# TimZaman/dotaclient

Hardware: NVIDIA H100
Metric: optimizer_steps_per_sec (higher is better)
Workload: dtype f32

## Files before the change

dotaclient_b200/_lib.py:

```python
import ctypes
import os

_HERE = os.path.dirname(os.path.abspath(__file__))
LIB_PATH = os.path.join(_HERE, "libdotaclient_b200.so")

_c = ctypes
_vp, _i32, _i64, _f32, _f64, _sz = _c.c_void_p, _c.c_int, _c.c_int64, _c.c_float, _c.c_double, _c.c_size_t
_ptr5 = _c.c_void_p * 5


class GatherDesc(_c.Structure):
    _fields_ = [("src", _vp), ("dst", _vp), ("outer", _i64), ("src_cols", _i64), ("row_bytes", _i64)]

SIGNATURES = {
    "dc_version": (_i32, []),
    "dc_last_error": (_c.c_char_p, []),
    "dc_device_info": (_i32, [_c.POINTER(_i32)] * 3),
    "dc_gae_scan": (_i32, [_vp, _i32, _vp, _vp, _i32, _vp, _vp, _f64, _f64, _vp, _vp, _vp]),
    "dc_vtrace_scan": (_i32, [_vp, _i32, _vp, _vp, _vp, _vp, _i32, _vp, _vp, _f64, _f64, _f64, _f64, _vp, _vp, _vp, _vp]),
    "dc_gather_columns": (_i32, [_c.POINTER(GatherDesc), _i32, _vp, _i64, _vp]),
    "dc_rnn_workspace_bytes": (_sz, [_i32, _i32, _i32]),
    "dc_rnn_seq_fwd": (_i32, [_i32, _vp, _vp, _vp, _vp, _vp, _i32, _i32, _i32, _vp, _vp]),
    "dc_rnn_seq_bwd": (_i32, [_i32, _vp, _vp, _vp, _vp, _vp, _vp, _vp, _vp, _vp, _i32, _i32, _i32, _vp, _vp]),
    "dc_rnn_seq_fwd_reset": (_i32, [_i32, _vp, _vp, _vp, _vp, _vp, _vp, _vp, _vp, _i32, _i32, _i32, _i32, _vp, _vp]),
    "dc_rnn_seq_bwd_reset": (_i32, [_i32, _vp, _vp, _vp, _vp, _vp, _vp, _vp, _vp, _vp, _vp, _vp, _i32, _i32, _i32, _i32, _vp,
                                    _vp]),
    "dc_gemm_tf32x3_supported": (_i32, [_i64, _i32, _i32]),
    "dc_gemm_tf32x3": (_i32, [_vp, _i32, _vp, _i32, _vp, _vp, _i32, _i64, _i32, _i32, _i32, _vp]),
    "dc_gemm_wgrad_workspace_bytes": (_sz, [_i32, _i32]),
    "dc_gemm_wgrad_tf32x3": (_i32, [_vp, _i32, _vp, _i32, _i64, _i32, _i32, _vp, _i32, _vp, _i32, _vp, _vp]),
    "dc_unit_basic_bwd_workspace_bytes": (_sz, []),
    "dc_env_fwd": (_i32, [_vp, _vp, _vp, _vp, _i32, _i64, _vp]),
    "dc_env_bwd_workspace_bytes": (_sz, []),
    "dc_env_bwd": (_i32, [_vp, _vp, _i32, _vp, _vp, _vp, _i64, _vp, _vp]),
    "dc_unit_wgrad_routed": (_i32, [_vp, _vp, _i32, _vp, _vp, _i64, _i32, _vp, _vp, _vp, _vp]),
    "dc_unit_dgrad_fused": (_i32, [_vp, _vp, _i32, _vp, _vp, _i32, _vp, _vp, _vp, _vp, _vp, _i64, _i32, _vp, _vp, _i32, _vp, _vp]),
    "dc_gemm_unit_max": (_i32, [_vp, _vp, _vp, _vp, _vp, _i32, _vp, _i64, _i32, _vp]),
    "dc_unit_embed_fwd": (_i32, [_vp, _vp, _vp, _vp, _vp, _vp, _vp, _vp, _i32, _vp, _i64, _i32, _vp]),
    "dc_target_unit_q_fwd": (_i32, [_vp, _i32, _c.c_void_p * 6, _vp, _vp, _vp, _i64, _vp]),
    "dc_target_unit_q_bwd": (_i32, [_vp, _c.c_void_p * 6, _vp, _vp, _vp, _i32, _i64, _vp]),
    "dc_ppo_loss_fwd_bwd": (_i32, [_ptr5, _ptr5, _ptr5, _vp, _vp, _vp, _vp, _i64, _f32, _f32, _f32, _ptr5, _vp, _vp,
                                   _vp, _vp, _vp]),
    "dc_ppo_loss_fwd_bwd_strided": (_i32, [_ptr5, _c.c_int64 * 5, _ptr5, _ptr5, _vp, _vp, _vp, _vp, _i64, _i64, _f32, _f32, _f32,
                                           _ptr5, _c.c_int64 * 5, _vp, _i64, _vp, _vp, _vp, _vp]),
    "dc_ppo_loss_fwd_bwd_dev": (_i32, [_ptr5, _c.c_int64 * 5, _ptr5, _ptr5, _vp, _vp, _vp, _vp, _i64, _vp, _i64, _vp,
                                       _ptr5, _c.c_int64 * 5, _vp, _i64, _vp, _vp, _vp, _vp, _vp]),
    "dc_ppo_loss_fwd_bwd_masked": (_i32, [_ptr5, _c.c_int64 * 5, _ptr5, _ptr5, _vp, _vp, _vp, _vp, _i64, _vp, _vp, _i64,
                                          _vp, _ptr5, _c.c_int64 * 5, _vp, _i64, _vp, _vp, _vp, _vp, _vp]),
    "dc_ppo_loss_fwd_bwd_joint": (_i32, [_ptr5, _c.c_int64 * 5, _ptr5, _ptr5, _vp, _vp, _vp, _vp, _i64, _vp, _vp, _i64,
                                         _vp, _ptr5, _c.c_int64 * 5, _vp, _i64, _vp, _vp, _vp, _vp, _vp]),
    "dc_selected_logp": (_i32, [_ptr5, _ptr5, _ptr5, _i64, _vp, _vp]),
    "dc_select_actions": (_i32, [_ptr5, _c.c_int64 * 5, _ptr5, _vp, _i64, _vp, _vp, _vp]),
    "dc_grad_flags": (_i32, [_vp, _i64, _vp, _i32, _vp, _vp]),
    "dc_grad_finish": (_i32, [_vp, _vp, _vp, _vp, _vp, _vp, _vp, _vp, _i32, _i64, _f64, _f64, _f64, _f64, _f64, _vp, _vp,
                              _vp, _vp]),
    "dc_grad_finish_dev": (_i32, [_vp, _vp, _vp, _vp, _vp, _vp, _vp, _vp, _i32, _i64, _vp, _f64, _f64, _f64, _vp, _vp, _vp,
                                  _vp]),
}

PPO_WORKSPACE_BYTES = 512
FINISH_WORKSPACE_BYTES = 1024
LOSS_SLOTS = 16
HPARAM_SLOTS = 8
HP_LR, HP_E_CLIP, HP_ENTROPY_COEF, HP_VF_COEF, HP_MAX_GRAD_NORM, HP_VALUE_CLIP = range(6)
PPO_STATS_SLOTS = 16
STAT_APPROX_KL, STAT_CLIP_FRACTION, STAT_EXPLAINED_VAR = 0, 6, 12
STAT_JOINT_APPROX_KL, STAT_JOINT_CLIP_FRACTION = 13, 14
VTRACE_STATS_SLOTS = 8
GATHER_MAX_TENSORS = 32
MAX_PARAM_TENSORS = 96

_lib = None


class NativeLibraryError(RuntimeError):
    pass


def load():
    global _lib
    if _lib is not None:
        return _lib
    if not os.path.exists(LIB_PATH):
        raise NativeLibraryError(
            "%s not found: build it with `python -m dotaclient_b200.build` (needs nvcc, sm_90a). "
            "dotaclient_b200 has no CPU fallback." % LIB_PATH)
    lib = ctypes.CDLL(LIB_PATH)
    for name, (res, args) in SIGNATURES.items():
        try:
            fn = getattr(lib, name)
        except AttributeError:
            continue
        fn.restype = res
        fn.argtypes = args
    _lib = lib
    return lib


def exported(name):
    lib = load()
    return hasattr(lib, name)


def check(rc, what):
    if rc != 0:
        msg = load().dc_last_error()
        raise RuntimeError("%s failed (code %d): %s" % (what, rc, msg.decode() if msg else "?"))


def ptr(t):
    return None if t is None else t.data_ptr()


def ptr5(tensors):
    return _ptr5(*[t.data_ptr() if t is not None else None for t in tensors])


def stream_ptr():
    import torch
    return torch.cuda.current_stream().cuda_stream
```

dotaclient_b200/csrc/capi.cu:

```cuda
#include <cstdarg>
#include <cstdio>
#include "dc_common.cuh"

static thread_local char g_err[512] = "";

void dc_set_error(const char *fmt, ...) {
    va_list ap;
    va_start(ap, fmt);
    vsnprintf(g_err, sizeof(g_err), fmt, ap);
    va_end(ap);
}

int dc_sm_count() {
    static int cached[64] = {0};
    int dev = 0;
    if (cudaGetDevice(&dev) != cudaSuccess || dev < 0 || dev >= 64) return 132;
    if (cached[dev] == 0) {
        int n = 0;
        if (cudaDeviceGetAttribute(&n, cudaDevAttrMultiProcessorCount, dev) != cudaSuccess || n <= 0) n = 132;
        cached[dev] = n;
    }
    return cached[dev];
}

extern "C" {

int dc_version(void) { return 107; }

const char *dc_last_error(void) { return g_err; }

int dc_device_info(int *sm_count, int *cc_major, int *cc_minor) {
    int dev = 0;
    DC_CUDA(cudaGetDevice(&dev));
    int v = 0;
    if (sm_count) { DC_CUDA(cudaDeviceGetAttribute(&v, cudaDevAttrMultiProcessorCount, dev)); *sm_count = v; }
    if (cc_major) { DC_CUDA(cudaDeviceGetAttribute(&v, cudaDevAttrComputeCapabilityMajor, dev)); *cc_major = v; }
    if (cc_minor) { DC_CUDA(cudaDeviceGetAttribute(&v, cudaDevAttrComputeCapabilityMinor, dev)); *cc_minor = v; }
    return DC_OK;
}

}
```

dotaclient_b200/csrc/gemm_tf32x3.cu:

```cuda
#include "dc_common.cuh"
#include "unit_basic.cuh"

namespace {

constexpr int BM = 128, BN = 128, BK = 32;
constexpr int kStages = 2;
constexpr int kTileBytes = BM * BK * 4;
constexpr int kStageBytes = 4 * kTileBytes;
constexpr int kProducerThreads = 128;
constexpr int kProducerGroups = kStages;
constexpr int kConsumerWarp0 = 4 * kProducerGroups;
constexpr int kConsumerThreads = 256;
constexpr int kThreads = kConsumerWarp0 * 32 + kConsumerThreads;
constexpr int kLdS = BN + 8;
constexpr int kDIn = kUnitFeatures;
constexpr size_t kOffStaging = (size_t)kStages * kStageBytes;
constexpr size_t kOffUnits = kOffStaging + (size_t)BM * kLdS * 4;
constexpr size_t kOffBars = kOffUnits + (size_t)BM * kDIn * 4;
constexpr size_t kSmemBytes = kOffBars + 128 + 1024 ;

#define DC_ACC8(b) "+f"(d[b]), "+f"(d[b + 1]), "+f"(d[b + 2]), "+f"(d[b + 3]), "+f"(d[b + 4]), "+f"(d[b + 5]), "+f"(d[b + 6]), "+f"(d[b + 7])
__device__ __forceinline__ void wgmma_m64n128k8(float (&d)[64], uint64_t desc_a, uint64_t desc_b) {
    asm volatile(
        "{\n\t.reg .pred p;\n\tsetp.ne.b32 p, %66, 0;\n\t"
        "wgmma.mma_async.sync.aligned.m64n128k8.f32.tf32.tf32 "
        "{%0, %1, %2, %3, %4, %5, %6, %7, %8, %9, %10, %11, %12, %13, %14, %15, "
        "%16, %17, %18, %19, %20, %21, %22, %23, %24, %25, %26, %27, %28, %29, %30, %31, "
        "%32, %33, %34, %35, %36, %37, %38, %39, %40, %41, %42, %43, %44, %45, %46, %47, "
        "%48, %49, %50, %51, %52, %53, %54, %55, %56, %57, %58, %59, %60, %61, %62, %63}, "
        "%64, %65, p, 1, 1;\n\t}\n"
        : DC_ACC8(0), DC_ACC8(8), DC_ACC8(16), DC_ACC8(24), DC_ACC8(32), DC_ACC8(40), DC_ACC8(48), DC_ACC8(56)
        : "l"(desc_a), "l"(desc_b), "r"(1));
}
#undef DC_ACC8

__device__ __forceinline__ void mma_stage(float (&d)[64], uint32_t stage_base, int wg) {
    const uint64_t a_hi = dc_wgmma_desc(stage_base + wg * (64 * 128)), a_lo = dc_wgmma_desc(stage_base + kTileBytes + wg * (64 * 128));
    const uint64_t b_hi = dc_wgmma_desc(stage_base + 2 * kTileBytes), b_lo = dc_wgmma_desc(stage_base + 3 * kTileBytes);
#pragma unroll
    for (int i = 0; i < 64; ++i) dc_reg_fence(d[i]);
    dc_wgmma_fence();
#pragma unroll
    for (int ks = 0; ks < BK / 8; ++ks) {
        const uint64_t adv = (uint64_t)(ks * 2);
        wgmma_m64n128k8(d, a_lo + adv, b_hi + adv);
        wgmma_m64n128k8(d, a_hi + adv, b_lo + adv);
        wgmma_m64n128k8(d, a_hi + adv, b_hi + adv);
    }
    dc_wgmma_commit();
    dc_wgmma_wait0();
#pragma unroll
    for (int i = 0; i < 64; ++i) dc_reg_fence(d[i]);
}

__device__ __forceinline__ void consume(float (&d)[64], unsigned char *tiles, uint64_t *full, uint64_t *empty, uint32_t &c, int n,
                                       int wg, int lane) {
#pragma unroll
    for (int i = 0; i < 64; ++i) d[i] = 0.f;
    for (int kc = 0; kc < n; ++kc, ++c) {
        const int s = c % kStages;
        dc_mbar_wait(&full[s], (c / kStages) & 1);
        __syncwarp();
        mma_stage(d, dc_smem_u32(tiles + (size_t)s * kStageBytes), wg);
        __syncwarp();
        if (lane == 0) dc_mbar_arrive(&empty[s]);
    }
}

__device__ __forceinline__ void consumer_sync() { asm volatile("bar.sync 1, %0;" ::"n"(kConsumerThreads) : "memory"); }

__device__ __forceinline__ void stage_acc(const float (&d)[64], float *S, int ct) {
    const int wg = ct >> 7, w = (ct >> 5) & 3, lane = ct & 31;
    const int r0 = 64 * wg + 16 * w + (lane >> 2), c0 = 2 * (lane & 3);
#pragma unroll
    for (int i = 0; i < 64; i += 2) {
        const int row = r0 + 8 * ((i >> 1) & 1), col = 8 * (i >> 2) + c0;
        *reinterpret_cast<float2 *>(S + row * kLdS + col) = make_float2(d[i], d[i + 1]);
    }
}

__device__ __forceinline__ void init_ring(uint64_t *bars) {
    if (threadIdx.x == 0) {
        for (int s = 0; s < kStages; ++s) { dc_mbar_init(&bars[s], 4); dc_mbar_init(&bars[kStages + s], kConsumerThreads / 32); }
        asm volatile("fence.mbarrier_init.release.cluster;" ::: "memory");
    }
    __syncthreads();
}
__device__ __forceinline__ unsigned char *smem_base(unsigned char *raw) {
    return reinterpret_cast<unsigned char *>((reinterpret_cast<uintptr_t>(raw) + 1023) & ~(uintptr_t)1023);
}
template <typename F>
__device__ __forceinline__ void produce(uint64_t *full, uint64_t *empty, uint32_t c, int lane, F &&store) {
    const int s = c % kStages;
    dc_mbar_wait(&empty[s], ((c / kStages) & 1) ^ 1);
    store(s);
    asm volatile("fence.proxy.async.shared::cta;" ::: "memory");
    __syncwarp();
    if (lane == 0) dc_mbar_arrive(&full[s]);
}

__device__ __forceinline__ void tile_load_k(const float *__restrict__ src, int ld, int row0, int rows_total, int k0, int t,
                                            float4 (&v)[8]) {
    const int c = t & 7, r0 = t >> 3;
#pragma unroll
    for (int i = 0; i < 8; ++i) {
        const int r = r0 + 16 * i;
        v[i] = (row0 + r < rows_total) ? __ldg(reinterpret_cast<const float4 *>(src + (size_t)(row0 + r) * ld + k0) + c)
                                       : make_float4(0.f, 0.f, 0.f, 0.f);
    }
}
__device__ __forceinline__ void tile_store_k(const float4 (&v)[8], unsigned char *dst_hi, unsigned char *dst_lo, int t) {
    const int c = t & 7, r0 = t >> 3;
#pragma unroll
    for (int i = 0; i < 8; ++i) {
        const int r = r0 + 16 * i;
        const int off = r * 128 + ((c ^ (r & 7)) << 4);
        float4 hi, lo;
        hi.x = dc_tf32_rna(v[i].x); hi.y = dc_tf32_rna(v[i].y); hi.z = dc_tf32_rna(v[i].z); hi.w = dc_tf32_rna(v[i].w);
        lo.x = v[i].x - hi.x; lo.y = v[i].y - hi.y; lo.z = v[i].z - hi.z; lo.w = v[i].w - hi.w;
        *reinterpret_cast<float4 *>(dst_hi + off) = hi;
        *reinterpret_cast<float4 *>(dst_lo + off) = lo;
    }
}

template <int NU>
struct DembRaw {
    static constexpr int kP = NU == 16 ? 1 : 2;
    static constexpr int kU = NU == 16 ? 8 : NU;
    float4 d[kP], d2[kP], a[kP];
    uint32_t am[kP];
    float g[kP][kU];
    bool ok[kP];
};
template <>
struct DembRaw<1> {
    float4 v[8];
};

template <int NU>
__device__ __forceinline__ void demb_fetch(DembRaw<NU> &raw, const float *__restrict__ dx, const float *__restrict__ dx2, int ld_dx,
                                           const uint8_t *__restrict__ argmax, const float *__restrict__ dl, int ld_dl,
                                           const float *__restrict__ att, int tok0, int n_tok, int k0, int t) {
    const float4 zero4 = make_float4(0.f, 0.f, 0.f, 0.f);
    if constexpr (NU == 1) {
        const int c = t & 7, r0 = t >> 3;
#pragma unroll
        for (int i = 0; i < 8; ++i) {
            const int n = tok0 + r0 + 16 * i;
            const bool ok = n < n_tok;
            const size_t nn = (size_t)min(n, n_tok - 1);
            float4 d = dx != nullptr ? __ldg(reinterpret_cast<const float4 *>(dx + nn * ld_dx + k0) + c) : zero4;
            if (dx2 != nullptr) {
                const float4 d2 = __ldg(reinterpret_cast<const float4 *>(dx2 + nn * ld_dx + k0) + c);
                d.x += d2.x; d.y += d2.y; d.z += d2.z; d.w += d2.w;
            }
            const float4 a4 = dl != nullptr ? __ldg(reinterpret_cast<const float4 *>(att + nn * 128 + k0) + c) : zero4;
            const float gl = dl != nullptr ? __ldg(dl + nn * ld_dl) : 0.f;
            raw.v[i] = ok ? make_float4(fmaf(gl, a4.x, d.x), fmaf(gl, a4.y, d.y), fmaf(gl, a4.z, d.z), fmaf(gl, a4.w, d.w)) : zero4;
        }
    } else {
        constexpr int kTileToks = (BM - BM % NU) / NU;
#pragma unroll
        for (int k = 0; k < DembRaw<NU>::kP; ++k) {
            const int p = t + kProducerThreads * k;
            const int c = p & 7, tokl = NU == 16 ? p >> 4 : p >> 3;
            const int u0 = NU == 16 ? ((p >> 3) & 1) * 8 : 0;
            const bool active = tokl < kTileToks;
            const int n = tok0 + tokl;
            raw.ok[k] = active && n < n_tok;
            const size_t nn = (size_t)min(n, n_tok - 1);
            float4 d = (active && dx != nullptr) ? __ldg(reinterpret_cast<const float4 *>(dx + nn * ld_dx + k0) + c) : zero4;
            const float4 d2 = (active && dx2 != nullptr) ? __ldg(reinterpret_cast<const float4 *>(dx2 + nn * ld_dx + k0) + c) : zero4;
            if constexpr (NU == 16) {
                raw.d2[k] = d2;
            } else {
                d.x += d2.x; d.y += d2.y; d.z += d2.z; d.w += d2.w;
            }
            raw.d[k] = d;
            raw.am[k] = (active && dx != nullptr) ? __ldg(reinterpret_cast<const uint32_t *>(argmax + nn * 128 + k0) + c) : 0u;
            raw.a[k] = (active && dl != nullptr) ? __ldg(reinterpret_cast<const float4 *>(att + nn * 128 + k0) + c) : zero4;
#pragma unroll
            for (int j = 0; j < DembRaw<NU>::kU; ++j) raw.g[k][j] = (active && dl != nullptr) ? __ldg(dl + nn * ld_dl + u0 + j) : 0.f;
        }
    }
}

__device__ __forceinline__ void store_hi_lo(unsigned char *dst_hi, unsigned char *dst_lo, int off, float4 o) {
    float4 hi, lo;
    hi.x = dc_tf32_rna(o.x); hi.y = dc_tf32_rna(o.y); hi.z = dc_tf32_rna(o.z); hi.w = dc_tf32_rna(o.w);
    lo.x = o.x - hi.x; lo.y = o.y - hi.y; lo.z = o.z - hi.z; lo.w = o.w - hi.w;
    *reinterpret_cast<float4 *>(dst_hi + off) = hi;
    *reinterpret_cast<float4 *>(dst_lo + off) = lo;
}

template <int NU>
__device__ __forceinline__ void demb_store(const DembRaw<NU> &raw, unsigned char *dst_hi, unsigned char *dst_lo, int t) {
    if constexpr (NU == 1) {
        tile_store_k(raw.v, dst_hi, dst_lo, t);
    } else {
        constexpr int kTileRows = BM - BM % NU, kTileToks = kTileRows / NU;
        const float4 zero4 = make_float4(0.f, 0.f, 0.f, 0.f);
#pragma unroll
        for (int k = 0; k < DembRaw<NU>::kP; ++k) {
            const int p = t + kProducerThreads * k;
            const int c = p & 7, tokl = NU == 16 ? p >> 4 : p >> 3;
            const int u0 = NU == 16 ? ((p >> 3) & 1) * 8 : 0;
            if (tokl < kTileToks) {
                float4 d = raw.d[k];
                if constexpr (NU == 16) { d.x += raw.d2[k].x; d.y += raw.d2[k].y; d.z += raw.d2[k].z; d.w += raw.d2[k].w; }
                const float4 a = raw.a[k];
                const uint32_t am = raw.am[k];
#pragma unroll
                for (int j = 0; j < DembRaw<NU>::kU; ++j) {
                    const int u = u0 + j, r = tokl * NU + u;
                    const float gl = raw.g[k][j];
                    float4 o;
                    o.x = fmaf(gl, a.x, (int)(am & 0xffu) == u ? d.x : 0.f);
                    o.y = fmaf(gl, a.y, (int)((am >> 8) & 0xffu) == u ? d.y : 0.f);
                    o.z = fmaf(gl, a.z, (int)((am >> 16) & 0xffu) == u ? d.z : 0.f);
                    o.w = fmaf(gl, a.w, (int)(am >> 24) == u ? d.w : 0.f);
                    store_hi_lo(dst_hi, dst_lo, r * 128 + ((c ^ (r & 7)) << 4), raw.ok[k] ? o : zero4);
                }
            }
        }
        if constexpr (kTileRows < BM) {
            if (t < (BM - kTileRows) * 8) {
                const int r = kTileRows + (t >> 3), c = t & 7;
                store_hi_lo(dst_hi, dst_lo, r * 128 + ((c ^ (r & 7)) << 4), zero4);
            }
        }
    }
}

__device__ __forceinline__ void store_row_k(const float (&v)[32], unsigned char *dst_hi, unsigned char *dst_lo, int row) {
#pragma unroll
    for (int c = 0; c < 8; ++c) {
        const int off = row * 128 + ((c ^ (row & 7)) << 4);
        float4 hi, lo;
        hi.x = dc_tf32_rna(v[4 * c]); hi.y = dc_tf32_rna(v[4 * c + 1]); hi.z = dc_tf32_rna(v[4 * c + 2]); hi.w = dc_tf32_rna(v[4 * c + 3]);
        lo.x = v[4 * c] - hi.x; lo.y = v[4 * c + 1] - hi.y; lo.z = v[4 * c + 2] - hi.z; lo.w = v[4 * c + 3] - hi.w;
        *reinterpret_cast<float4 *>(dst_hi + off) = hi;
        *reinterpret_cast<float4 *>(dst_lo + off) = lo;
    }
}

__global__ void __launch_bounds__(kThreads, 1) gemm_tf32x3_kernel(const float *__restrict__ A, int lda,
                                                                  const float *__restrict__ B, int ldb,
                                                                  const float *__restrict__ bias, float *__restrict__ C,
                                                                  int ldc, int M, int N, int K, int relu, int ksplit,
                                                                  long long c_split_stride) {
    constexpr int kTileRows = BM;
    extern __shared__ unsigned char smem_raw[];
    unsigned char *tiles = smem_base(smem_raw);
    float *S = reinterpret_cast<float *>(tiles + kOffStaging);
    uint64_t *full = reinterpret_cast<uint64_t *>(tiles + kOffBars), *empty = full + kStages;

    const int warp = threadIdx.x >> 5, lane = threadIdx.x & 31;
    const int m_blocks = (M + kTileRows - 1) / kTileRows, n_blocks = (N + BN - 1) / BN, k_chunks = K / BK / ksplit;
    const int tiles_mn = m_blocks * n_blocks, tiles_total = tiles_mn * ksplit;
    init_ring(full);

    if (warp < kConsumerWarp0) {
        const int t = threadIdx.x & (kProducerThreads - 1), g = warp >> 2;
        uint32_t c = 0;
        for (int tile = blockIdx.x; tile < tiles_total; tile += gridDim.x) {
            const int tmn = tile % tiles_mn, kc0 = (tile / tiles_mn) * k_chunks;
            const int m0 = (tmn / n_blocks) * kTileRows, n0 = (tmn % n_blocks) * BN;
            for (int kc = 0; kc < k_chunks; ++kc, ++c) {
                if ((int)(c % kProducerGroups) != g) continue;
                float4 va[8], vb[8];
                tile_load_k(A, lda, m0, M, (kc0 + kc) * BK, t, va);
                tile_load_k(B, ldb, n0, N, (kc0 + kc) * BK, t, vb);
                produce(full, empty, c, lane, [&](int s) {
                    unsigned char *st = tiles + (size_t)s * kStageBytes;
                    tile_store_k(va, st, st + kTileBytes, t);
                    tile_store_k(vb, st + 2 * kTileBytes, st + 3 * kTileBytes, t);
                });
            }
        }
    } else {
        const int ct = threadIdx.x - kConsumerWarp0 * 32, wg = ct >> 7, cw = ct >> 5;
        float d[64];
        uint32_t c = 0;
        for (int tile = blockIdx.x; tile < tiles_total; tile += gridDim.x) {
            const int tmn = tile % tiles_mn, sp = tile / tiles_mn;
            const int m0 = (tmn / n_blocks) * kTileRows, n0 = (tmn % n_blocks) * BN;
            consume(d, tiles, full, empty, c, k_chunks, wg, lane);
            consumer_sync();
            stage_acc(d, S, ct);
            consumer_sync();
            const bool lane_in = n0 + 4 * lane < N;
            const bool has_bias = bias != nullptr && sp == 0 && lane_in;
            const float4 b4 = has_bias ? __ldg(reinterpret_cast<const float4 *>(bias + n0) + lane) : make_float4(0.f, 0.f, 0.f, 0.f);
            float *cbase = C + (size_t)sp * (size_t)c_split_stride + n0 + 4 * lane;
            for (int r = cw; lane_in && r < BM && m0 + r < M; r += kConsumerThreads / 32) {
                float4 v = *reinterpret_cast<const float4 *>(S + r * kLdS + 4 * lane);
                if (has_bias) { v.x += b4.x; v.y += b4.y; v.z += b4.z; v.w += b4.w; }
                if (relu) { v.x = fmaxf(v.x, 0.f); v.y = fmaxf(v.y, 0.f); v.z = fmaxf(v.z, 0.f); v.w = fmaxf(v.w, 0.f); }
                *reinterpret_cast<float4 *>(cbase + (size_t)(m0 + r) * ldc) = v;
            }
        }
    }
}

constexpr int kWsRows = 64;
constexpr int kWsStages = 8;
constexpr int kWsChunkBytes = kWsRows * BK * 4;
constexpr int kWsThreads = kConsumerThreads + 128;
constexpr int kWsLdS = 40;
constexpr size_t kWsOffRing = (size_t)4 * 2 * kTileBytes;
constexpr size_t kWsOffStaging = kWsOffRing + (size_t)kWsStages * kWsChunkBytes;
constexpr size_t kWsOffBars = kWsOffStaging + (size_t)(kConsumerThreads / 32) * 16 * kWsLdS * 4;
constexpr size_t kWsSmemBytes = kWsOffBars + 2 * kWsStages * 8 + 1024 ;
constexpr size_t kWsOffUnits = kWsOffBars + 2 * kWsStages * 8;
constexpr size_t kWsGenSmemBytes = kWsOffUnits + (size_t)4 * kWsRows * kDIn * 4 + 1024 ;
static_assert(kWsSmemBytes <= 227 * 1024 && kWsGenSmemBytes <= 227 * 1024, "weight-stationary GEMM exceeds the shared-memory opt-in");
static_assert(kWsOffUnits % 16 == 0, "unit rows are staged with 16-byte stores");

struct GenA {
    const float *units, *w_b, *b_b;
    float *basic_out;
};

__device__ __forceinline__ void cp_async16(uint32_t dst, const void *src, uint32_t src_bytes) {
    asm volatile("cp.async.cg.shared.global [%0], [%1], 16, %2;" ::"r"(dst), "l"(src), "r"(src_bytes) : "memory");
}
__device__ __forceinline__ void cp_async_arrive(uint64_t *bar) {
    asm volatile("cp.async.mbarrier.arrive.noinc.shared::cta.b64 [%0];" ::"r"(dc_smem_u32(bar)) : "memory");
}

#define DC_ACC8(b) "+f"(d[b]), "+f"(d[b + 1]), "+f"(d[b + 2]), "+f"(d[b + 3]), "+f"(d[b + 4]), "+f"(d[b + 5]), "+f"(d[b + 6]), "+f"(d[b + 7])
__device__ __forceinline__ void wgmma_m64n128k8_rs(float (&d)[64], uint32_t a0, uint32_t a1, uint32_t a2, uint32_t a3, uint64_t desc_b) {
    asm volatile(
        "{\n\t.reg .pred p;\n\tsetp.ne.b32 p, %69, 0;\n\t"
        "wgmma.mma_async.sync.aligned.m64n128k8.f32.tf32.tf32 "
        "{%0, %1, %2, %3, %4, %5, %6, %7, %8, %9, %10, %11, %12, %13, %14, %15, "
        "%16, %17, %18, %19, %20, %21, %22, %23, %24, %25, %26, %27, %28, %29, %30, %31, "
        "%32, %33, %34, %35, %36, %37, %38, %39, %40, %41, %42, %43, %44, %45, %46, %47, "
        "%48, %49, %50, %51, %52, %53, %54, %55, %56, %57, %58, %59, %60, %61, %62, %63}, "
        "{%64, %65, %66, %67}, %68, p, 1, 1;\n\t}\n"
        : DC_ACC8(0), DC_ACC8(8), DC_ACC8(16), DC_ACC8(24), DC_ACC8(32), DC_ACC8(40), DC_ACC8(48), DC_ACC8(56)
        : "r"(a0), "r"(a1), "r"(a2), "r"(a3), "l"(desc_b), "r"(1));
}
#undef DC_ACC8

__device__ __forceinline__ void ws_fetch(float (&v)[16], const float *chunk, int rlo, int rhi, bool hi_ok, int q) {
#pragma unroll
    for (int ks = 0; ks < BK / 8; ++ks) {
#pragma unroll
        for (int h = 0; h < 2; ++h) {
            const int j = 2 * ks + h;
            v[4 * ks + 2 * h] = chunk[rlo * BK + ((j ^ (rlo & 7)) << 2) + q];
            v[4 * ks + 2 * h + 1] = hi_ok ? chunk[rhi * BK + ((j ^ (rhi & 7)) << 2) + q] : 0.f;
        }
    }
}

template <int NU, bool kGenA>
__global__ void __launch_bounds__(kWsThreads, 1) gemm_ws_kernel(const float *__restrict__ A, int lda,
                                                                const float *__restrict__ B, int ldb,
                                                                const float *__restrict__ bias, float *__restrict__ C,
                                                                int ldc, int M, int N, int K, int relu,
                                                                float *__restrict__ C_copy, uint8_t *__restrict__ argmax, GenA gen) {
    constexpr int kWarpRows = NU == 5 ? 15 : 16;
    constexpr int kTileRows = 4 * kWarpRows;
    extern __shared__ unsigned char smem_raw[];
    unsigned char *sm = smem_base(smem_raw);
    unsigned char *ring = sm + kWsOffRing;
    uint64_t *full = reinterpret_cast<uint64_t *>(sm + kWsOffBars), *empty = full + kWsStages;

    const int warp = threadIdx.x >> 5, lane = threadIdx.x & 31;
    const int n_blocks = (N + BN - 1) / BN, m_blocks = (M + kTileRows - 1) / kTileRows, k_chunks = K / BK;
    const int n0 = (blockIdx.x % n_blocks) * BN, mb0 = blockIdx.x / n_blocks, mstride = gridDim.x / n_blocks;
    if (threadIdx.x == 0) {
        for (int s = 0; s < kWsStages; ++s) { dc_mbar_init(&full[s], kGenA ? 1 : 128); dc_mbar_init(&empty[s], 4); }
        asm volatile("fence.mbarrier_init.release.cluster;" ::: "memory");
    }
    __syncthreads();

    if constexpr (kGenA) if (warp >= kConsumerThreads / 32) {
        const int kc = warp - kConsumerThreads / 32, ch = lane & 7, r0 = lane >> 3;
        const int j0 = kc * BK + 4 * ch;
        float wb[4][kDIn], bb[4];
#pragma unroll
        for (int e = 0; e < 4; ++e) {
            bb[e] = __ldg(gen.b_b + j0 + e);
#pragma unroll
            for (int k = 0; k < kDIn; ++k) wb[e][k] = __ldg(gen.w_b + (j0 + e) * kDIn + k);
        }
        float4 *su = reinterpret_cast<float4 *>(sm + kWsOffUnits) + kc * (kWsRows * kDIn / 4);
        const float4 *units4 = reinterpret_cast<const float4 *>(gen.units);
        constexpr int kU4 = kWsRows * kDIn / 4 / 32;
        float4 nxt[kU4];
        auto fetch = [&](int mb) {
            const bool live = mb < m_blocks;
            const int m0 = live ? mb * kTileRows : 0;
#pragma unroll
            for (int i = 0; i < kU4; ++i) {
                const int idx = lane + 32 * i, r = idx / 3;
                nxt[i] = (live && r < kTileRows && m0 + r < M) ? __ldg(units4 + (size_t)m0 * 3 + idx) : make_float4(0.f, 0.f, 0.f, 0.f);
            }
        };
        fetch(mb0);
        uint32_t c = kc;
        for (int mb = mb0; mb < m_blocks; mb += mstride, c += 4) {
            const int m0 = mb * kTileRows;
            __syncwarp();
#pragma unroll
            for (int i = 0; i < kU4; ++i) su[lane + 32 * i] = nxt[i];
            __syncwarp();
            fetch(mb + mstride);
            const int s = c % kWsStages;
            dc_mbar_wait(&empty[s], ((c / kWsStages) & 1) ^ 1);
            unsigned char *chunk = ring + (size_t)s * kWsChunkBytes;
#pragma unroll 4
            for (int i = 0; i < kWsRows / 4; ++i) {
                const int r = r0 + 4 * i;
                const bool ok = r < kTileRows && m0 + r < M;
                const float4 u0 = su[3 * r], u1 = su[3 * r + 1], u2 = su[3 * r + 2];
                const float u[kDIn] = {u0.x, u0.y, u0.z, u0.w, u1.x, u1.y, u1.z, u1.w, u2.x, u2.y, u2.z, u2.w};
                float4 v = make_float4(dc_unit_basic(u, wb[0], bb[0]), dc_unit_basic(u, wb[1], bb[1]), dc_unit_basic(u, wb[2], bb[2]),
                                       dc_unit_basic(u, wb[3], bb[3]));
                if (!ok) v = make_float4(0.f, 0.f, 0.f, 0.f);
                *reinterpret_cast<float4 *>(chunk + r * 128 + ((ch ^ (r & 7)) << 4)) = v;
                if (gen.basic_out != nullptr && ok) *reinterpret_cast<float4 *>(gen.basic_out + (size_t)(m0 + r) * BN + j0) = v;
            }
            __syncwarp();
            if (lane == 0) dc_mbar_arrive(&full[s]);
        }
        return;
    }
    if constexpr (!kGenA) if (warp >= kConsumerThreads / 32) {
        const int p = threadIdx.x - kConsumerThreads, ch = p & 7;
        uint32_t c = 0;
        for (int mb = mb0; mb < m_blocks; mb += mstride) {
            const int m0 = mb * kTileRows;
            for (int kc = 0; kc < k_chunks; ++kc, ++c) {
                const int s = c % kWsStages;
                dc_mbar_wait(&empty[s], ((c / kWsStages) & 1) ^ 1);
                const uint32_t dst = dc_smem_u32(ring + (size_t)s * kWsChunkBytes);
#pragma unroll
                for (int i = 0; i < kWsRows / 16; ++i) {
                    const int r = (p >> 3) + 16 * i;
                    const bool ok = r < kTileRows && m0 + r < M;
                    const float *src = A + (ok ? (size_t)(m0 + r) * lda : 0) + kc * BK + 4 * ch;
                    cp_async16(dst + r * 128 + ((ch ^ (r & 7)) << 4), src, ok ? 16u : 0u);
                }
                cp_async_arrive(&full[s]);
            }
        }
        asm volatile("cp.async.wait_all;" ::: "memory");
        return;
    }

    const int wg = warp >> 2, w4 = warp & 3, t = threadIdx.x & 127, q = lane & 3, g8 = lane >> 2;
    {
        for (int kc = wg; kc < k_chunks; kc += 2) {
            float4 vb[8];
            tile_load_k(B, ldb, n0, N, kc * BK, t, vb);
            tile_store_k(vb, sm + (size_t)kc * 2 * kTileBytes, sm + (size_t)kc * 2 * kTileBytes + kTileBytes, t);
        }
        asm volatile("fence.proxy.async.shared::cta;" ::: "memory");
        consumer_sync();
    }
    const uint32_t w_base = dc_smem_u32(sm);
    const int rlo = kWarpRows * w4 + g8, rhi = rlo + 8;
    const bool hi_ok = NU != 5 || g8 < 7;
    float *Sw = reinterpret_cast<float *>(sm + kWsOffStaging) + warp * 16 * kWsLdS;
    float d[64];
    uint32_t c = 0;
    int i = 0;
    for (int mb = mb0; mb < m_blocks; mb += mstride, ++i, c += k_chunks) {
        if ((i & 1) != wg) continue;
        const int m0 = mb * kTileRows;
#pragma unroll
        for (int j = 0; j < 64; ++j) d[j] = 0.f;
        float v[16];
        uint32_t ahi[16], alo[16];
        {
            const int s = c % kWsStages;
            dc_mbar_wait(&full[s], (c / kWsStages) & 1);
            ws_fetch(v, reinterpret_cast<const float *>(ring + (size_t)s * kWsChunkBytes), rlo, rhi, hi_ok, q);
        }
        for (int kc = 0; kc < k_chunks; ++kc) {
#pragma unroll
            for (int j = 0; j < 16; ++j) {
                const float h = dc_tf32_rna(v[j]);
                ahi[j] = __float_as_uint(h);
                alo[j] = __float_as_uint(v[j] - h);
            }
            __syncwarp();
            if (lane == 0) dc_mbar_arrive(&empty[(c + kc) % kWsStages]);
#pragma unroll
            for (int j = 0; j < 64; ++j) dc_reg_fence(d[j]);
            dc_wgmma_fence();
            const uint64_t b_hi = dc_wgmma_desc(w_base + kc * 2 * kTileBytes), b_lo = dc_wgmma_desc(w_base + kc * 2 * kTileBytes + kTileBytes);
#pragma unroll
            for (int ks = 0; ks < BK / 8; ++ks) {
                const uint64_t adv = (uint64_t)(ks * 2);
                wgmma_m64n128k8_rs(d, alo[4 * ks], alo[4 * ks + 1], alo[4 * ks + 2], alo[4 * ks + 3], b_hi + adv);
                wgmma_m64n128k8_rs(d, ahi[4 * ks], ahi[4 * ks + 1], ahi[4 * ks + 2], ahi[4 * ks + 3], b_lo + adv);
                wgmma_m64n128k8_rs(d, ahi[4 * ks], ahi[4 * ks + 1], ahi[4 * ks + 2], ahi[4 * ks + 3], b_hi + adv);
            }
            dc_wgmma_commit();
            if (kc + 1 < k_chunks) {
                const uint32_t cn = c + kc + 1;
                const int s = cn % kWsStages;
                dc_mbar_wait(&full[s], (cn / kWsStages) & 1);
                ws_fetch(v, reinterpret_cast<const float *>(ring + (size_t)s * kWsChunkBytes), rlo, rhi, hi_ok, q);
            }
            dc_wgmma_wait0();
#pragma unroll
            for (int j = 0; j < 16; ++j) asm volatile("" : "+r"(ahi[j]), "+r"(alo[j])::"memory");
#pragma unroll
            for (int j = 0; j < 64; ++j) dc_reg_fence(d[j]);
        }

        if constexpr (NU == 0) {
            const int row_lo = m0 + rlo, row_hi = m0 + rhi;
            float *c_lo = row_lo < M ? C + (size_t)row_lo * ldc : nullptr, *c_hi = row_hi < M ? C + (size_t)row_hi * ldc : nullptr;
#pragma unroll
            for (int g = 0; g < BN / 8; ++g) {
                const int col = n0 + 8 * g + 2 * q;
                if (col >= N) break;
                const float2 b2 = bias != nullptr ? __ldg(reinterpret_cast<const float2 *>(bias + col)) : make_float2(0.f, 0.f);
                float2 lo = make_float2(d[4 * g], d[4 * g + 1]), hi = make_float2(d[4 * g + 2], d[4 * g + 3]);
                if (bias != nullptr) { lo.x += b2.x; lo.y += b2.y; hi.x += b2.x; hi.y += b2.y; }
                if (relu) { lo.x = fmaxf(lo.x, 0.f); lo.y = fmaxf(lo.y, 0.f); hi.x = fmaxf(hi.x, 0.f); hi.y = fmaxf(hi.y, 0.f); }
                if (c_lo) *reinterpret_cast<float2 *>(c_lo + col) = lo;
                if (c_hi) *reinterpret_cast<float2 *>(c_hi + col) = hi;
            }
        } else {
            constexpr int kToks = kWarpRows / NU;
            const int tok0 = m0 / NU + kToks * w4, n_tok = M / NU;
#pragma unroll
            for (int b = 0; b < BN / 32; ++b) {
#pragma unroll
                for (int g = 0; g < 4; ++g) {
                    const int j = 4 * (4 * b + g);
                    *reinterpret_cast<float2 *>(Sw + g8 * kWsLdS + 8 * g + 2 * q) = make_float2(d[j], d[j + 1]);
                    *reinterpret_cast<float2 *>(Sw + (g8 + 8) * kWsLdS + 8 * g + 2 * q) = make_float2(d[j + 2], d[j + 3]);
                }
                __syncwarp();
                const int col = 32 * b + lane;
                const float bias_f = __ldg(bias + col);
#pragma unroll
                for (int tk = 0; tk < kToks; ++tk) {
                    const int tok = tok0 + tk;
                    if (tok >= n_tok) break;
                    const float *p = Sw + tk * NU * kWsLdS + lane;
                    float best = p[0];
                    int best_u = 0;
#pragma unroll
                    for (int u = 1; u < NU; ++u) {
                        const float x = p[u * kWsLdS];
                        if (x > best) { best = x; best_u = u; }
                    }
                    const float o = best + bias_f;
                    C[(size_t)tok * ldc + col] = o;
                    if (C_copy) C_copy[(size_t)tok * ldc + col] = o;
                    argmax[(size_t)tok * BN + col] = (uint8_t)best_u;
                }
                __syncwarp();
            }
        }
    }
}

template <int NU>
__global__ void __launch_bounds__(kThreads, 1) unit_dgrad_fused_kernel(const float *__restrict__ dx, const float *__restrict__ dx2, int ld_dx,
                                                                       const uint8_t *__restrict__ argmax,
                                                                       const float *__restrict__ dl, int ld_dl,
                                                                       const float *__restrict__ att,
                                                                       const float *__restrict__ Wt, const float *__restrict__ units,
                                                                       const float *__restrict__ w_b, const float *__restrict__ b_b,
                                                                       int n_tok, float *__restrict__ partial) {
    constexpr int kTileRows = BM - BM % NU, kTileToks = kTileRows / NU;
    constexpr int k_chunks = BN / BK;
    extern __shared__ unsigned char smem_raw[];
    unsigned char *tiles = smem_base(smem_raw);
    float *S = reinterpret_cast<float *>(tiles + kOffStaging);
    float *U = reinterpret_cast<float *>(tiles + kOffUnits);
    uint64_t *full = reinterpret_cast<uint64_t *>(tiles + kOffBars), *empty = full + kStages;

    const int warp = threadIdx.x >> 5, lane = threadIdx.x & 31;
    const int M = n_tok * NU;
    const int m_blocks = (M + kTileRows - 1) / kTileRows;
    init_ring(full);

    if (warp < kConsumerWarp0) {
        const int t = threadIdx.x & (kProducerThreads - 1), g = warp >> 2;
        uint32_t c = 0;
        for (int mb = blockIdx.x; mb < m_blocks; mb += gridDim.x) {
            const int tok0 = mb * kTileToks;
            for (int kc = 0; kc < k_chunks; ++kc, ++c) {
                if ((int)(c % kProducerGroups) != g) continue;
                DembRaw<NU> raw;
                float4 vb[8];
                demb_fetch<NU>(raw, dx, dx2, ld_dx, argmax, dl, ld_dl, att, tok0, n_tok, kc * BK, t);
                tile_load_k(Wt, BN, 0, BN, kc * BK, t, vb);
                produce(full, empty, c, lane, [&](int s) {
                    unsigned char *st = tiles + (size_t)s * kStageBytes;
                    demb_store<NU>(raw, st, st + kTileBytes, t);
                    tile_store_k(vb, st + 2 * kTileBytes, st + 3 * kTileBytes, t);
                });
            }
        }
    } else {
        const int ct = threadIdx.x - kConsumerWarp0 * 32, wg = ct >> 7;
        const int col = ct & (BN - 1), half = ct >> 7;
        float wb[kDIn];
#pragma unroll
        for (int k = 0; k < kDIn; ++k) wb[k] = __ldg(w_b + col * kDIn + k);
        const float bb = __ldg(b_b + col);
        float acc[kDIn];
#pragma unroll
        for (int k = 0; k < kDIn; ++k) acc[k] = 0.f;
        float accb = 0.f;
        float d[64];
        uint32_t c = 0;
        for (int mb = blockIdx.x; mb < m_blocks; mb += gridDim.x) {
            const int m0 = mb * kTileRows, rows_valid = min(kTileRows, M - m0);
            consume(d, tiles, full, empty, c, k_chunks, wg, lane);
            consumer_sync();
            stage_acc(d, S, ct);
            const float4 *usrc = reinterpret_cast<const float4 *>(units + (size_t)m0 * kDIn);
            for (int i = ct; i < rows_valid * (kDIn / 4); i += kConsumerThreads) reinterpret_cast<float4 *>(U)[i] = __ldg(usrc + i);
            consumer_sync();
            const int r_end = min(64 * half + 64, rows_valid);
            for (int r = 64 * half; r < r_end; ++r) {
                const float4 *up = reinterpret_cast<const float4 *>(U + r * kDIn);
                const float4 u0 = up[0], u1 = up[1], u2 = up[2];
                const float u[kDIn] = {u0.x, u0.y, u0.z, u0.w, u1.x, u1.y, u1.z, u1.w, u2.x, u2.y, u2.z, u2.w};
                const float gval = dc_unit_basic(u, wb, bb) > 0.f ? S[r * kLdS + col] : 0.f;
#pragma unroll
                for (int k = 0; k < kDIn; ++k) acc[k] = fmaf(gval, u[k], acc[k]);
                accb += gval;
            }
        }
        float *prow = partial + ((size_t)(blockIdx.x * 2 + half) * BN + col) * (kDIn + 1);
#pragma unroll
        for (int k = 0; k < kDIn; ++k) prow[k] = acc[k];
        prow[kDIn] = accb;
    }
}

constexpr int kWgStages = 4;
constexpr int kWgLdX = BN + 8;
constexpr int kWgStageBytes = 2 * kTileBytes + BK * kWgLdX * 4;
constexpr size_t kWgOffColsum = (size_t)kWgStages * kWgStageBytes;
constexpr size_t kWgOffBars = kWgOffColsum + 2 * BM * 4;
constexpr size_t kWgSmemBytes = kWgOffBars + 2 * kWgStages * 8 + 1024 ;
static_assert(kWgStageBytes % 1024 == 0, "the swizzled dY^T tiles need 1024-byte aligned slots");
static_assert(kWgSmemBytes <= 227 * 1024, "weight-gradient GEMM exceeds the shared-memory opt-in");

__device__ __forceinline__ void wgmma_wait1() { asm volatile("wgmma.wait_group.sync.aligned 1;" ::: "memory"); }
__device__ __forceinline__ float lds_f32(uint32_t addr) {
    float v;
    asm volatile("ld.shared.f32 %0, [%1];" : "=f"(v) : "r"(addr) : "memory");
    return v;
}

template <int NU>
__global__ void __launch_bounds__(kThreads, 1) gemm_wgrad_kernel(const float *__restrict__ dY, int ldy,
                                                                 const float *__restrict__ dY2,
                                                                 const uint8_t *__restrict__ argmax,
                                                                 const float *__restrict__ X, int ldx, int T, int No,
                                                                 int Ni, int nsplit, float *__restrict__ part_w,
                                                                 float *__restrict__ part_b) {
    constexpr int kTPC = NU > 0 ? BK / NU : 0;
    constexpr int kRPC = NU > 0 ? kTPC * NU : BK;
    extern __shared__ unsigned char smem_raw[];
    unsigned char *ring = smem_base(smem_raw);
    float *colsum_s = reinterpret_cast<float *>(ring + kWgOffColsum);
    uint64_t *full = reinterpret_cast<uint64_t *>(ring + kWgOffBars), *empty = full + kWgStages;

    const int warp = threadIdx.x >> 5, lane = threadIdx.x & 31;
    const int n_blocks = (Ni + BN - 1) / BN, tiles_mn = ((No + BM - 1) / BM) * n_blocks;
    const int tile = blockIdx.x % tiles_mn, split = blockIdx.x / tiles_mn;
    const int m0 = (tile / n_blocks) * BM, n0 = (tile % n_blocks) * BN;
    const int chunks_total = (T + kRPC - 1) / kRPC;
    const int my_chunks = split < chunks_total ? (chunks_total - split + nsplit - 1) / nsplit : 0;
    if (threadIdx.x == 0) {
        for (int s = 0; s < kWgStages; ++s) { dc_mbar_init(&full[s], kProducerThreads + 4); dc_mbar_init(&empty[s], kConsumerThreads / 32); }
        asm volatile("fence.mbarrier_init.release.cluster;" ::: "memory");
    }
    __syncthreads();

    if (warp < kConsumerWarp0) {
        const int g = warp >> 2, t = threadIdx.x & (kProducerThreads - 1), o = m0 + t;
        const bool o_in = o < No;
        const int xc = t & 31;
        const bool xc_in = n0 + 4 * xc < Ni;
        float cs = 0.f;
        for (int j = g; j < my_chunks; j += kProducerGroups) {
            float va[32];
            if constexpr (NU > 0) {
                const int tok0 = (split + j * nsplit) * kTPC, n_tok = T / NU;
                float dv[kTPC];
                int am[kTPC];
#pragma unroll
                for (int k = 0; k < kTPC; ++k) {
                    const bool ok = tok0 + k < n_tok;
                    const size_t at = (size_t)(tok0 + k) * ldy + o;
                    dv[k] = ok ? __ldg(dY + at) : 0.f;
                    if (ok && dY2 != nullptr) dv[k] += __ldg(dY2 + at);
                    am[k] = ok ? (int)__ldg(argmax + (size_t)(tok0 + k) * 128 + o) : 255;
                }
#pragma unroll
                for (int i = 0; i < 32; ++i) va[i] = (i < kRPC && am[i / NU] == i % NU) ? dv[i / NU] : 0.f;
            } else {
                const int t0 = (split + j * nsplit) * BK;
                const float *p = dY + (size_t)t0 * ldy + o;
#pragma unroll
                for (int i = 0; i < 32; ++i) va[i] = (o_in && t0 + i < T) ? __ldg(p + (size_t)i * ldy) : 0.f;
            }
#pragma unroll
            for (int i = 0; i < 32; ++i) cs += va[i];
            const int t0 = (split + j * nsplit) * kRPC, tend = min(T, t0 + kRPC);
            const int s = j % kWgStages;
            dc_mbar_wait(&empty[s], ((j / kWgStages) & 1) ^ 1);
            unsigned char *st = ring + (size_t)s * kWgStageBytes;
            const uint32_t xs = dc_smem_u32(st + 2 * kTileBytes);
#pragma unroll
            for (int r = 0; r < BK / 4; ++r) {
                const int row = (t >> 5) + 4 * r;
                const bool ok = xc_in && t0 + row < tend;
                cp_async16(xs + (row * kWgLdX + 4 * xc) * 4, X + (ok ? (size_t)(t0 + row) * ldx + n0 + 4 * xc : 0), ok ? 16u : 0u);
            }
            cp_async_arrive(&full[s]);
            store_row_k(va, st, st + kTileBytes, t);
            asm volatile("fence.proxy.async.shared::cta;" ::: "memory");
            __syncwarp();
            if (lane == 0) dc_mbar_arrive(&full[s]);
        }
        colsum_s[g * 128 + t] = cs;
        asm volatile("cp.async.wait_all;" ::: "memory");
    } else {
        const int ct = threadIdx.x - kConsumerWarp0 * 32, wg = ct >> 7, w4 = (ct >> 5) & 3, q = lane & 3;
        const int rlo = 64 * wg + 16 * w4 + (lane >> 2);
        float d[64];
#pragma unroll
        for (int i = 0; i < 64; ++i) d[i] = 0.f;
        uint32_t ahi[2][4] = {}, alo[2][4] = {};
#pragma unroll
        for (int i = 0; i < 64; ++i) dc_reg_fence(d[i]);
        for (int j = 0; j < my_chunks; ++j) {
            const int s = j % kWgStages;
            dc_mbar_wait(&full[s], (j / kWgStages) & 1);
            const uint32_t st = dc_smem_u32(ring + (size_t)s * kWgStageBytes);
            const uint32_t xk = st + 2 * kTileBytes + (q * kWgLdX + rlo) * 4;
            float v[16];
#pragma unroll
            for (int ks = 0; ks < BK / 8; ++ks) {
                const uint32_t x8 = xk + 8 * ks * kWgLdX * 4;
                v[4 * ks] = lds_f32(x8);
                v[4 * ks + 1] = lds_f32(x8 + 8 * 4);
                v[4 * ks + 2] = lds_f32(x8 + 4 * kWgLdX * 4);
                v[4 * ks + 3] = lds_f32(x8 + (4 * kWgLdX + 8) * 4);
            }
            const uint64_t b_hi = dc_wgmma_desc(st), b_lo = dc_wgmma_desc(st + kTileBytes);
#pragma unroll
            for (int ks = 0; ks < BK / 8; ++ks) {
                const int b = ks & 1;
#pragma unroll
                for (int e = 0; e < 4; ++e) {
                    const float h = dc_tf32_rna(v[4 * ks + e]);
                    ahi[b][e] = __float_as_uint(h);
                    alo[b][e] = __float_as_uint(v[4 * ks + e] - h);
                }
                dc_wgmma_fence();
                const uint64_t adv = (uint64_t)(ks * 2);
                wgmma_m64n128k8_rs(d, ahi[b][0], ahi[b][1], ahi[b][2], ahi[b][3], b_lo + adv);
                wgmma_m64n128k8_rs(d, alo[b][0], alo[b][1], alo[b][2], alo[b][3], b_hi + adv);
                wgmma_m64n128k8_rs(d, ahi[b][0], ahi[b][1], ahi[b][2], ahi[b][3], b_hi + adv);
                dc_wgmma_commit();
                wgmma_wait1();
#pragma unroll
                for (int e = 0; e < 4; ++e) asm volatile("" : "+r"(ahi[b ^ 1][e]), "+r"(alo[b ^ 1][e])::"memory");
                if (ks == 0 && j > 0) {
                    __syncwarp();
                    if (lane == 0) dc_mbar_arrive(&empty[(j - 1) % kWgStages]);
                }
            }
        }
        dc_wgmma_wait0();
#pragma unroll
        for (int i = 0; i < 64; ++i) dc_reg_fence(d[i]);
        float *pt = part_w + ((size_t)split * tiles_mn + tile) * BM * BN + rlo;
#pragma unroll
        for (int k = 0; k < 64; ++k) pt[(size_t)(8 * (k >> 2) + 2 * q + (k & 1)) * BN + 8 * ((k >> 1) & 1)] = d[k];
    }
    __syncthreads();
    if (part_b != nullptr && n0 == 0 && threadIdx.x < 128 && m0 + (int)threadIdx.x < No)
        part_b[(size_t)split * No + m0 + threadIdx.x] = colsum_s[threadIdx.x] + colsum_s[128 + threadIdx.x];
}

constexpr int kRedRows = 8;
__global__ void __launch_bounds__(32 * kRedRows) wgrad_reduce_kernel(const float *__restrict__ part_w, const float *__restrict__ part_b,
                                                                     int nsplit, int No, int Ni, float *__restrict__ dW, int ldw,
                                                                     float *__restrict__ db, int accumulate) {
    __shared__ float4 sh[kRedRows][32];
    const int x = threadIdx.x & 31, y = threadIdx.x >> 5;
    const int n_blocks = (Ni + BN - 1) / BN, tiles_mn = ((No + BM - 1) / BM) * n_blocks;
    const int total4 = No * Ni / 4, bias4 = db != nullptr ? No / 4 : 0;
    const int idx = blockIdx.x * 32 + x;
    const float *src = nullptr;
    float *dst = nullptr;
    size_t stride = 0;
    if (idx < total4) {
        const int o = (idx * 4) / Ni, i = (idx * 4) % Ni;
        const int tile = (o / BM) * n_blocks + i / BN;
        src = part_w + ((size_t)tile * BM + o % BM) * BN + i % BN;
        stride = (size_t)tiles_mn * BM * BN;
        dst = dW + (size_t)o * ldw + i;
    } else if (idx < total4 + bias4) {
        src = part_b + (size_t)(idx - total4) * 4;
        stride = (size_t)No;
        dst = db + (size_t)(idx - total4) * 4;
    }
    float4 acc = make_float4(0.f, 0.f, 0.f, 0.f);
    if (src != nullptr) {
#pragma unroll 4
        for (int s = y; s < nsplit; s += kRedRows) {
            const float4 v = __ldg(reinterpret_cast<const float4 *>(src + (size_t)s * stride));
            acc.x += v.x; acc.y += v.y; acc.z += v.z; acc.w += v.w;
        }
    }
    sh[y][x] = acc;
    __syncthreads();
    if (y == 0 && dst != nullptr) {
        float4 t = accumulate ? *reinterpret_cast<const float4 *>(dst) : make_float4(0.f, 0.f, 0.f, 0.f);
#pragma unroll
        for (int r = 0; r < kRedRows; ++r) { t.x += sh[r][x].x; t.y += sh[r][x].y; t.z += sh[r][x].z; t.w += sh[r][x].w; }
        *reinterpret_cast<float4 *>(dst) = t;
    }
}

}

extern "C" int dc_gemm_tf32x3_supported(int64_t M, int N, int K) { return M > 0 && N > 0 && K > 0 && N % 32 == 0 && K % BK == 0; }

template <int NU, bool kGenA = false>
static int launch_ws(const float *A, int lda, const float *B, int ldb, const float *bias, float *C, int ldc, int M, int N,
                     int K, int relu, float *C_copy, uint8_t *argmax, cudaStream_t st, GenA gen = GenA{}) {
    const int tile_rows = NU == 5 ? 60 : kWsRows;
    const int n_blocks = (N + BN - 1) / BN, m_blocks = (M + tile_rows - 1) / tile_rows;
    int per_block = dc_sm_count() / n_blocks;
    if (per_block < 1) per_block = 1;
    if (per_block > m_blocks) per_block = m_blocks;
    const size_t smem = kGenA ? kWsGenSmemBytes : kWsSmemBytes;
    DC_CUDA(cudaFuncSetAttribute(gemm_ws_kernel<NU, kGenA>, cudaFuncAttributeMaxDynamicSharedMemorySize, (int)smem));
    gemm_ws_kernel<NU, kGenA><<<n_blocks * per_block, kWsThreads, smem, st>>>(A, lda, B, ldb, bias, C, ldc, M, N, K, relu, C_copy,
                                                                             argmax, gen);
    DC_LAUNCH_OK();
    return DC_OK;
}

extern "C" int dc_gemm_tf32x3(const float *A, int lda, const float *B, int ldb, const float *bias, float *C, int ldc,
                              int64_t M, int N, int K, int relu, dc_stream_t stream) {
    DC_REQUIRE(A && B && C, DC_EINVAL, "dc_gemm_tf32x3: null pointer");
    DC_REQUIRE(dc_gemm_tf32x3_supported(M, N, K) && M < (1ll << 31) - BM, DC_EUNSUPPORTED,
               "dc_gemm_tf32x3: need N %% 32 == 0 and K %% 32 == 0 (M=%lld N=%d K=%d)", (long long)M, N, K);
    DC_REQUIRE(lda >= K && ldb >= K && ldc >= N && lda % 4 == 0 && ldb % 4 == 0 && ldc % 4 == 0, DC_EINVAL,
               "dc_gemm_tf32x3: leading dimensions must be >= extent and multiples of 4 floats");
    DC_REQUIRE(((uintptr_t)A & 15) == 0 && ((uintptr_t)B & 15) == 0 && ((uintptr_t)C & 15) == 0 && (!bias || ((uintptr_t)bias & 15) == 0),
               DC_EINVAL, "dc_gemm_tf32x3: pointers must be 16-byte aligned");
    if (K <= 4 * BK) return launch_ws<0>(A, lda, B, ldb, bias, C, ldc, (int)M, N, K, relu, nullptr, nullptr, dc_cu_stream(stream));
    const int tiles = (int)((M + BM - 1) / BM) * ((N + BN - 1) / BN);
    DC_CUDA(cudaFuncSetAttribute(gemm_tf32x3_kernel, cudaFuncAttributeMaxDynamicSharedMemorySize, (int)kSmemBytes));
    const int grid = tiles < dc_sm_count() ? tiles : dc_sm_count();
    gemm_tf32x3_kernel<<<grid, kThreads, kSmemBytes, dc_cu_stream(stream)>>>(A, lda, B, ldb, bias, C, ldc, (int)M, N, K, relu, 1, 0);
    DC_LAUNCH_OK();
    return DC_OK;
}

int dc_gemm_tf32x3_splitk(const float *A, int lda, const float *B, int ldb, float *part, int64_t M, int N, int K, int ksplit,
                          bool first_call, cudaStream_t st) {
    DC_REQUIRE(A && B && part && ksplit >= 1 && N % BN == 0 && K % (BK * ksplit) == 0 && M > 0, DC_EINVAL,
               "dc_gemm_tf32x3_splitk: bad arguments (M=%lld N=%d K=%d ksplit=%d)", (long long)M, N, K, ksplit);
    if (first_call)
        DC_CUDA(cudaFuncSetAttribute(gemm_tf32x3_kernel, cudaFuncAttributeMaxDynamicSharedMemorySize, (int)kSmemBytes));
    const int tiles = (int)((M + BM - 1) / BM) * (N / BN) * ksplit;
    const int grid = tiles < dc_sm_count() ? tiles : dc_sm_count();
    gemm_tf32x3_kernel<<<grid, kThreads, kSmemBytes, st>>>(A, lda, B, ldb, nullptr, part, N, (int)M, N, K, 0, ksplit, (long long)M * N);
    DC_LAUNCH_OK();
    return DC_OK;
}

static int wgrad_tiles(int No, int Ni) { return ((No + BM - 1) / BM) * ((Ni + BN - 1) / BN); }

static int wgrad_splits(int No, int Ni) {
    const int tiles_mn = wgrad_tiles(No, Ni);
    const int n = dc_sm_count() / tiles_mn;
    return n < 1 ? 1 : n;
}

extern "C" size_t dc_gemm_wgrad_workspace_bytes(int No, int Ni) {
    if (No <= 0 || Ni <= 0 || No % 32 || Ni % 32) return 0;
    const int nsplit = wgrad_splits(No, Ni);
    return ((size_t)nsplit * wgrad_tiles(No, Ni) * BM * BN + (size_t)nsplit * No) * sizeof(float);
}

extern "C" int dc_gemm_wgrad_tf32x3(const float *dY, int ldy, const float *X, int ldx, int64_t T, int No, int Ni, float *dW,
                                    int ldw, float *db, int accumulate, void *workspace, dc_stream_t stream) {
    DC_REQUIRE(dY && X && dW && workspace, DC_EINVAL, "dc_gemm_wgrad_tf32x3: null pointer");
    DC_REQUIRE(T > 0 && T < (1ll << 31) - BK && No > 0 && Ni > 0 && No % 32 == 0 && Ni % 32 == 0, DC_EUNSUPPORTED,
               "dc_gemm_wgrad_tf32x3: need No %% 32 == 0 and Ni %% 32 == 0 (T=%lld No=%d Ni=%d)", (long long)T, No, Ni);
    DC_REQUIRE(ldy >= No && ldx >= Ni && ldw >= Ni && ldy % 4 == 0 && ldx % 4 == 0 && ldw % 4 == 0, DC_EINVAL,
               "dc_gemm_wgrad_tf32x3: bad leading dimension");
    DC_REQUIRE(((uintptr_t)dY & 15) == 0 && ((uintptr_t)X & 15) == 0 && ((uintptr_t)dW & 15) == 0 && ((uintptr_t)workspace & 15) == 0 &&
                   ((uintptr_t)db & 15) == 0,
               DC_EINVAL, "dc_gemm_wgrad_tf32x3: pointers must be 16-byte aligned");
    const int tiles_mn = wgrad_tiles(No, Ni), nsplit = wgrad_splits(No, Ni);
    float *part_w = reinterpret_cast<float *>(workspace);
    float *part_b = db ? part_w + (size_t)nsplit * tiles_mn * BM * BN : nullptr;
    cudaStream_t st = dc_cu_stream(stream);
    DC_CUDA(cudaFuncSetAttribute(gemm_wgrad_kernel<0>, cudaFuncAttributeMaxDynamicSharedMemorySize, (int)kWgSmemBytes));
    gemm_wgrad_kernel<0><<<tiles_mn * nsplit, kThreads, kWgSmemBytes, st>>>(dY, ldy, nullptr, nullptr, X, ldx, (int)T, No, Ni,
                                                                                      nsplit, part_w, part_b);
    DC_LAUNCH_OK();
    const int total4 = No * Ni / 4 + (db ? No / 4 : 0);
    wgrad_reduce_kernel<<<(total4 + 31) / 32, 32 * kRedRows, 0, st>>>(part_w, part_b, nsplit, No, Ni, dW, ldw, db, accumulate);
    DC_LAUNCH_OK();
    return DC_OK;
}

extern "C" int dc_gemm_unit_max(const float *basic, const float *w, const float *bias, float *xmax, float *xmax_copy, int ld_x,
                                uint8_t *argmax, int64_t n_tokens, int n_units, dc_stream_t stream) {
    DC_REQUIRE(basic && w && bias && xmax && argmax && n_tokens > 0, DC_EINVAL, "dc_gemm_unit_max: null pointer / empty input");
    DC_REQUIRE(n_units == 5 || n_units == 16, DC_EUNSUPPORTED, "dc_gemm_unit_max: n_units=%d (5 or 16; 1-unit groups are plain GEMMs)", n_units);
    DC_REQUIRE(ld_x >= BN && n_tokens * n_units < (1ll << 31) - BM, DC_EINVAL, "dc_gemm_unit_max: bad ld_x / size");
    DC_REQUIRE(((uintptr_t)basic & 15) == 0 && ((uintptr_t)w & 15) == 0, DC_EINVAL, "dc_gemm_unit_max: pointers must be 16-byte aligned");
    const int M = (int)(n_tokens * n_units);
    cudaStream_t st = dc_cu_stream(stream);
    if (n_units == 5) return launch_ws<5>(basic, BN, w, BN, bias, xmax, ld_x, M, BN, BN, 0, xmax_copy, argmax, st);
    return launch_ws<16>(basic, BN, w, BN, bias, xmax, ld_x, M, BN, BN, 0, xmax_copy, argmax, st);
}

extern "C" int dc_unit_embed_fwd(const float *units, const float *w_b, const float *b_b, float *basic_out, const float *w, const float *bias,
                                 float *xmax, float *xmax_copy, int ld_x, uint8_t *argmax, int64_t n_tokens, int n_units,
                                 dc_stream_t stream) {
    DC_REQUIRE(units && w_b && b_b && w && bias && xmax && n_tokens > 0, DC_EINVAL, "dc_unit_embed_fwd: null pointer / empty input");
    DC_REQUIRE(n_units == 1 || n_units == 5 || n_units == 16, DC_EUNSUPPORTED, "dc_unit_embed_fwd: n_units=%d (1, 5 or 16)", n_units);
    DC_REQUIRE(n_units == 1 ? (argmax == nullptr && xmax_copy == nullptr) : argmax != nullptr, DC_EINVAL,
               "dc_unit_embed_fwd: the arg-max (and the copy) go with the max-pool of n_units 5 and 16 only");
    DC_REQUIRE(ld_x >= BN && ld_x % 4 == 0 && n_tokens * n_units < (1ll << 31) - BM, DC_EINVAL, "dc_unit_embed_fwd: bad ld_x / size");
    DC_REQUIRE(((uintptr_t)units & 15) == 0 && ((uintptr_t)basic_out & 15) == 0 && ((uintptr_t)w & 15) == 0 && ((uintptr_t)bias & 15) == 0 &&
                   ((uintptr_t)xmax & 15) == 0 && ((uintptr_t)xmax_copy & 15) == 0,
               DC_EINVAL, "dc_unit_embed_fwd: units, basic_out, w, bias, xmax, xmax_copy must be 16-byte aligned");
    const int M = (int)(n_tokens * n_units);
    const GenA gen{units, w_b, b_b, basic_out};
    cudaStream_t st = dc_cu_stream(stream);
    if (n_units == 1) return launch_ws<0, true>(nullptr, BN, w, BN, bias, xmax, ld_x, M, BN, BN, 0, nullptr, nullptr, st, gen);
    if (n_units == 5) return launch_ws<5, true>(nullptr, BN, w, BN, bias, xmax, ld_x, M, BN, BN, 0, xmax_copy, argmax, st, gen);
    return launch_ws<16, true>(nullptr, BN, w, BN, bias, xmax, ld_x, M, BN, BN, 0, xmax_copy, argmax, st, gen);
}

extern "C" int dc_unit_dgrad_fused(const float *d_xmax, const float *d_xmax2, int ld_dx, const uint8_t *argmax, const float *dlogits,
                                   int ld_dl, const float *att, const float *w_t, const float *units, const float *w_b,
                                   const float *b_b, int64_t n_tokens, int n_units, float *dw_b, float *db_b, int accumulate,
                                   void *workspace, dc_stream_t stream) {
    DC_REQUIRE(w_t && units && w_b && b_b && dw_b && db_b && workspace && n_tokens > 0, DC_EINVAL, "dc_unit_dgrad_fused: null pointer / empty input");
    DC_REQUIRE(n_units == 1 || n_units == 5 || n_units == 16, DC_EUNSUPPORTED, "dc_unit_dgrad_fused: n_units=%d (1, 5 or 16)", n_units);
    DC_REQUIRE((d_xmax == nullptr && d_xmax2 == nullptr) || (d_xmax != nullptr && ld_dx >= BN && ld_dx % 4 == 0), DC_EINVAL,
               "dc_unit_dgrad_fused: bad d_xmax / ld_dx");
    DC_REQUIRE(d_xmax == nullptr || n_units == 1 || argmax != nullptr, DC_EINVAL, "dc_unit_dgrad_fused: routing needs the arg-max");
    DC_REQUIRE((dlogits == nullptr) == (att == nullptr) && (dlogits == nullptr || ld_dl >= n_units), DC_EINVAL,
               "dc_unit_dgrad_fused: dlogits and att come together");
    DC_REQUIRE(n_tokens * n_units < (1ll << 31) - BM, DC_EINVAL, "dc_unit_dgrad_fused: too many rows");
    DC_REQUIRE(((uintptr_t)d_xmax & 15) == 0 && ((uintptr_t)d_xmax2 & 15) == 0 && ((uintptr_t)argmax & 3) == 0 && ((uintptr_t)att & 15) == 0 &&
                   ((uintptr_t)w_t & 15) == 0 && ((uintptr_t)units & 15) == 0 && ((uintptr_t)workspace & 15) == 0,
               DC_EINVAL, "dc_unit_dgrad_fused: d_xmax, att, w_t, units must be 16-byte aligned (arg-max 4-byte)");
    const int n_tok = (int)n_tokens;
    const int tile_rows = BM - BM % n_units;
    int grid = (int)((n_tokens * n_units + tile_rows - 1) / tile_rows);
    if (grid > dc_sm_count()) grid = dc_sm_count();
    float *partial = reinterpret_cast<float *>(workspace);
    cudaStream_t st = dc_cu_stream(stream);
#define DC_LAUNCH_DGRAD(NU)                                                                                                          \
    do {                                                                                                                              \
        DC_CUDA(cudaFuncSetAttribute(unit_dgrad_fused_kernel<NU>, cudaFuncAttributeMaxDynamicSharedMemorySize, (int)kSmemBytes)); \
        unit_dgrad_fused_kernel<NU><<<grid, kThreads, kSmemBytes, st>>>(d_xmax, d_xmax2, ld_dx, argmax, dlogits, ld_dl, att, w_t,    \
                                                                            units, w_b, b_b, n_tok, partial);                        \
    } while (0)
    if (n_units == 1) DC_LAUNCH_DGRAD(1);
    else if (n_units == 5) DC_LAUNCH_DGRAD(5);
    else DC_LAUNCH_DGRAD(16);
#undef DC_LAUNCH_DGRAD
    DC_LAUNCH_OK();
    return dc_unit_basic_reduce(partial, 2 * grid, dw_b, db_b, accumulate, st);
}

extern "C" int dc_unit_wgrad_routed(const float *d_xmax, const float *d_xmax2, int ld_dx, const uint8_t *argmax, const float *basic,
                                    int64_t n_tokens, int n_units, float *dW, float *db, void *workspace, dc_stream_t stream) {
    DC_REQUIRE(d_xmax && argmax && basic && dW && db && workspace && n_tokens > 0, DC_EINVAL, "dc_unit_wgrad_routed: null pointer / empty input");
    DC_REQUIRE(n_units == 5 || n_units == 16, DC_EUNSUPPORTED, "dc_unit_wgrad_routed: n_units=%d (5 or 16; a 1-unit group is dc_gemm_wgrad_tf32x3)", n_units);
    DC_REQUIRE(ld_dx >= BM && n_tokens * n_units < (1ll << 31) - BK, DC_EINVAL, "dc_unit_wgrad_routed: bad ld_dx / size");
    DC_REQUIRE(((uintptr_t)basic & 15) == 0 && ((uintptr_t)dW & 15) == 0 && ((uintptr_t)db & 15) == 0 && ((uintptr_t)workspace & 15) == 0,
               DC_EINVAL, "dc_unit_wgrad_routed: pointers must be 16-byte aligned");
    const int No = BM, Ni = BN, nsplit = wgrad_splits(No, Ni);
    const int T = (int)(n_tokens * n_units);
    float *part_w = reinterpret_cast<float *>(workspace);
    float *part_b = part_w + (size_t)nsplit * No * Ni;
    cudaStream_t st = dc_cu_stream(stream);
    if (n_units == 5) {
        DC_CUDA(cudaFuncSetAttribute(gemm_wgrad_kernel<5>, cudaFuncAttributeMaxDynamicSharedMemorySize, (int)kWgSmemBytes));
        gemm_wgrad_kernel<5><<<nsplit, kThreads, kWgSmemBytes, st>>>(d_xmax, ld_dx, d_xmax2, argmax, basic, BN, T, No, Ni, nsplit,
                                                                                part_w, part_b);
    } else {
        DC_CUDA(cudaFuncSetAttribute(gemm_wgrad_kernel<16>, cudaFuncAttributeMaxDynamicSharedMemorySize, (int)kWgSmemBytes));
        gemm_wgrad_kernel<16><<<nsplit, kThreads, kWgSmemBytes, st>>>(d_xmax, ld_dx, d_xmax2, argmax, basic, BN, T, No, Ni, nsplit,
                                                                                 part_w, part_b);
    }
    DC_LAUNCH_OK();
    wgrad_reduce_kernel<<<(No * Ni / 4 + No / 4 + 31) / 32, 32 * kRedRows, 0, st>>>(part_w, part_b, nsplit, No, Ni, dW, Ni, db, 0);
    DC_LAUNCH_OK();
    return DC_OK;
}
```

dotaclient_b200/encoder_ops.py:

```python
import torch

from . import _lib
from .ops import PROFILE, _f32c, _need_cuda, gemm_tf32x3, gemm_wgrad_supported

UNITS = (1, 5, 16, 16, 1, 1)
OFFSETS = (0, 1, 6, 22, 38, 39)
MAX_UNITS = 40
C = 128
XCAT = 7 * C

_basic_ws = {}


def _basic_workspace(device):
    ws = _basic_ws.get(device)
    if ws is None:
        ws = torch.empty(int(_lib.load().dc_unit_basic_bwd_workspace_bytes()), dtype=torch.uint8, device=device)
        _basic_ws[device] = ws
    return ws


_env_ws = {}


def _env_workspace(device):
    ws = _env_ws.get(device)
    if ws is None:
        ws = torch.empty(int(_lib.load().dc_env_bwd_workspace_bytes()), dtype=torch.uint8, device=device)
        _env_ws[device] = ws
    return ws


_wgrad_ws = {}


def _wgrad_workspace(No, Ni, device):
    key = (No, Ni, device)
    ws = _wgrad_ws.get(key)
    if ws is None:
        ws = torch.empty(int(_lib.load().dc_gemm_wgrad_workspace_bytes(No, Ni)), dtype=torch.uint8, device=device)
        _wgrad_ws[key] = ws
    return ws




def _ptr(t, float_offset=0):
    return t.data_ptr() + 4 * float_offset


def _ptr6(tensors):
    return (_lib._c.c_void_p * 6)(*[t.data_ptr() for t in tensors])


class UnitEncoder(torch.autograd.Function):

    @staticmethod
    def forward(ctx, link, wait, need_grad, env, w_e, b_e, w_b, b_b, *rest):
        units, weights, biases = rest[:6], rest[6:12], rest[12:18]
        ctx.link = link
        _need_cuda(env, w_b, *units)
        lib = _lib.load()
        st = _lib.stream_ptr()
        lead = units[0].shape[:-2]
        N = 1
        for d in lead:
            N *= d
        dev = units[0].device
        w_b, b_b = _f32c(w_b.detach()), _f32c(b_b.detach())
        units = [_f32c(u.detach()).reshape(N * n, 12) for u, n in zip(units, UNITS)]
        units = [u if u.data_ptr() % 16 == 0 else u.clone() for u in units]
        weights = [_f32c(w.detach()) for w in weights]
        biases = [_f32c(b.detach()) for b in biases]
        xcat = torch.empty((N, XCAT), dtype=torch.float32, device=dev)
        argmax = torch.zeros((5, N, C), dtype=torch.uint8, device=dev)
        env2 = _f32c(env.detach()).reshape(N, 3)
        w_e, b_e = _f32c(w_e.detach()), _f32c(b_e.detach())
        if wait is not None:
            wait(env2)
        with PROFILE.span("env_fwd", 1, 4 * N * (3 + C)):
            _lib.check(lib.dc_env_fwd(env2.data_ptr(), w_e.data_ptr(), b_e.data_ptr(), xcat.data_ptr(), XCAT, N, st), "dc_env_fwd")
        basics = []
        for g, n_u in enumerate(UNITS):
            R = N * n_u
            if wait is not None:
                wait(units[g])
            if g == 5:
                continue
            basic = torch.empty((R, C), dtype=torch.float32, device=dev) if need_grad else None
            copy = _ptr(xcat, 6 * C) if g == 3 else None
            am = argmax[g].data_ptr() if n_u > 1 else None
            nbytes = 4 * (R * 12 + (R * C if need_grad else 0) + C * C + N * C) + (N * C if n_u > 1 else 0)
            with PROFILE.span("gemm_unit_max" if n_u > 1 else "gemm_tf32x3", 1, nbytes):
                _lib.check(lib.dc_unit_embed_fwd(units[g].data_ptr(), w_b.data_ptr(), b_b.data_ptr(), _lib.ptr(basic),
                                                 weights[g].data_ptr(), biases[g].data_ptr(), _ptr(xcat, (g + 1) * C), copy, XCAT,
                                                 am, N, n_u, st), "dc_unit_embed_fwd")
            basics.append(basic)
        link["units"], link["w_b"], link["b_b"] = units, w_b, b_b
        link["weights"], link["biases"] = weights, biases
        ctx.N = N
        ctx.lead = lead
        ctx.save_for_backward(argmax, *units, *basics, *weights, env2, xcat, w_b, b_b)
        return xcat.view(*lead, XCAT)

    @staticmethod
    def backward(ctx, d_xcat):
        saved = ctx.saved_tensors
        argmax, units, basics, weights, env2, xcat = saved[0], saved[1:7], saved[7:12], saved[12:18], saved[18], saved[19]
        w_b, b_b = saved[20], saved[21]
        N = ctx.N
        lib = _lib.load()
        st = _lib.stream_ptr()
        dev = argmax.device
        pending = ctx.link.pop("pending", None)
        d_xcat = _f32c(d_xcat).reshape(N, XCAT)
        dw_e = torch.empty((C, 3), dtype=torch.float32, device=dev)
        db_e = torch.empty(C, dtype=torch.float32, device=dev)
        with PROFILE.span("env_bwd", 2, 4 * N * (2 * C + 3)):
            _lib.check(lib.dc_env_bwd(d_xcat.data_ptr(), xcat.data_ptr(), XCAT, env2.data_ptr(), dw_e.data_ptr(), db_e.data_ptr(),
                                      N, _env_workspace(dev).data_ptr(), st), "dc_env_bwd")
        dl = att = s_head = None
        if pending is not None:
            dl, att, s_head = pending
        dw_b = torch.empty((C, 12), dtype=torch.float32, device=dev)
        db_b = torch.empty(C, dtype=torch.float32, device=dev)
        dw_all = torch.zeros((6, C, C), dtype=torch.float32, device=dev)
        db_all = torch.zeros((6, C), dtype=torch.float32, device=dev)
        ws_w = _wgrad_workspace(C, C, dev)
        ws_b = _basic_workspace(dev)
        for g, (n_u, off) in enumerate(zip(UNITS, OFFSETS)):
            R = N * n_u
            routed = g < 5
            dx = _ptr(d_xcat, (g + 1) * C) if routed else None
            dx2 = _ptr(d_xcat, 6 * C) if g == 3 else None
            if routed and n_u > 1:
                with PROFILE.span("gemm_wgrad", 2, 4 * (R * C + C * C + N * C) + N * C):
                    _lib.check(lib.dc_unit_wgrad_routed(dx, dx2, XCAT, argmax[g].data_ptr(), basics[g].data_ptr(), N, n_u,
                                                        dw_all[g].data_ptr(), db_all[g].data_ptr(), ws_w.data_ptr(), st),
                               "dc_unit_wgrad_routed")
            elif routed:
                with PROFILE.span("gemm_wgrad", 2, 4 * (2 * R * C + C * C)):
                    _lib.check(lib.dc_gemm_wgrad_tf32x3(dx, XCAT, basics[g].data_ptr(), C, R, C, C, dw_all[g].data_ptr(), C,
                                                        db_all[g].data_ptr(), 0, ws_w.data_ptr(), st), "dc_gemm_wgrad_tf32x3")
            wt = weights[g].t().contiguous()
            with PROFILE.span("unit_dgrad_fused", 2, N * (4 * C + C) * (1 if routed else 0) + 4 * R * 12 + (4 * N * (C + n_u) if dl is not None else 0)):
                _lib.check(lib.dc_unit_dgrad_fused(dx, dx2, XCAT, argmax[g].data_ptr() if (routed and n_u > 1) else None,
                                                   None if dl is None else _ptr(dl, off), MAX_UNITS, None if att is None else att.data_ptr(),
                                                   wt.data_ptr(), units[g].data_ptr(), w_b.data_ptr(), b_b.data_ptr(), N, n_u,
                                                   dw_b.data_ptr(), db_b.data_ptr(), 1 if g > 0 else 0, ws_b.data_ptr(), st),
                           "dc_unit_dgrad_fused")
        if dl is not None:
            dw_head = torch.empty((C, QW), dtype=torch.float32, device=dev)
            with PROFILE.span("gemm_wgrad", 2, 4 * (N * C + N * QW + C * QW)):
                _lib.check(lib.dc_gemm_wgrad_tf32x3(att.data_ptr(), C, s_head.data_ptr(), QW, N, C, QW, dw_head.data_ptr(), QW, None, 0,
                                                    _wgrad_workspace(C, QW, dev).data_ptr(), st), "dc_gemm_wgrad_tf32x3")
            dw_all += dw_head[:, :6 * C].reshape(C, 6, C).permute(1, 0, 2)
            db_all += dw_head[:, 6 * C:6 * C + 6].t()
        dws, dbs = list(dw_all.unbind(0)), list(db_all.unbind(0))
        return (None, None, None, None, dw_e, db_e, dw_b, db_b) + (None,) * 6 + tuple(dws) + tuple(dbs)


QW = 7 * C


class TargetUnit(torch.autograd.Function):

    @staticmethod
    def forward(ctx, att, link):
        _need_cuda(att)
        units, w_b, b_b = link["units"], link["w_b"], link["b_b"]
        weights, biases = link["weights"], link["biases"]
        lead = att.shape[:-1]
        N = att.numel() // C
        att2 = _f32c(att.detach()).reshape(N, C)
        dev = att2.device
        bias_block = torch.zeros((C, C), dtype=torch.float32, device=dev)
        bias_block[:, :6] = torch.stack(biases, dim=1)
        bm = torch.cat(list(weights) + [bias_block], dim=1)
        q = gemm_tf32x3(att2, bm.t().contiguous())
        logits = torch.empty((N, MAX_UNITS), dtype=torch.float32, device=dev)
        with PROFILE.span("target_unit_fwd", 1, 4 * N * (MAX_UNITS * 12 + QW + MAX_UNITS)):
            _lib.check(_lib.load().dc_target_unit_q_fwd(q.data_ptr(), QW, _ptr6(units), w_b.data_ptr(), b_b.data_ptr(),
                                                        logits.data_ptr(), N, _lib.stream_ptr()), "dc_target_unit_q_fwd")
        ctx.save_for_backward(att2, bm, w_b, b_b, *units)
        ctx.link = link
        ctx.att_shape = att.shape
        return logits.view(*lead, MAX_UNITS)

    @staticmethod
    def backward(ctx, dlogits):
        att2, bm, w_b, b_b = ctx.saved_tensors[:4]
        units = ctx.saved_tensors[4:]
        N = att2.shape[0]
        dl = _f32c(dlogits).reshape(N, MAX_UNITS)
        s = torch.empty((N, QW), dtype=torch.float32, device=att2.device)
        with PROFILE.span("target_unit_bwd", 1):
            _lib.check(_lib.load().dc_target_unit_q_bwd(dl.data_ptr(), _ptr6(units), w_b.data_ptr(), b_b.data_ptr(), s.data_ptr(),
                                                        QW, N, _lib.stream_ptr()), "dc_target_unit_q_bwd")
        d_att = gemm_tf32x3(s, bm)
        ctx.link["pending"] = (dl, att2, s)
        return d_att.view(ctx.att_shape), None


def unit_encoder(env, w_e, b_e, w_b, b_b, units, weights, biases, wait=None):
    link = {}
    tensors = (env, w_e, b_e, w_b, b_b, *units, *weights, *biases)
    need_grad = torch.is_grad_enabled() and any(t.requires_grad for t in tensors)
    xcat = UnitEncoder.apply(link, wait, need_grad, *tensors)
    return link, xcat


def target_unit(att, link):
    return TargetUnit.apply(att, link)


__all__ = ["unit_encoder", "target_unit", "gemm_wgrad_supported"]
```

include/dotaclient_b200.h:

```cpp
#ifndef DOTACLIENT_B200_H
#define DOTACLIENT_B200_H

#include <stddef.h>
#include <stdint.h>

#ifdef __cplusplus
extern "C" {
#endif

#define DC_OK 0
#define DC_EINVAL (-1)
#define DC_EUNSUPPORTED (-2)

#define DC_CELL_GRU 0
#define DC_CELL_LSTM 1

#define DC_NUM_HEADS 5
#define DC_LOSS_SLOTS 16

typedef void *dc_stream_t;

int dc_version(void);
const char *dc_last_error(void);
int dc_device_info(int *sm_count, int *cc_major, int *cc_minor);

int dc_gae_scan(const float *rewards, int n_sub, const float *values, const int64_t *seg_off,
                int n_seg, const float *boot_value, const float *boot_reward, double gamma,
                double lam, float *adv, float *ret, dc_stream_t stream);

#define DC_VTRACE_STATS_SLOTS 8
int dc_vtrace_scan(const float *rewards, int n_sub, const float *values, const float *logp_target,
                   const float *logp_behaviour, const int64_t *seg_off, int n_seg, const int64_t *valid_len,
                   const float *boot_value, double gamma, double lam, double rho_clip, double c_clip, float *pg_adv,
                   float *vs, double *seg_stats, dc_stream_t stream);

typedef struct {
    const void *src;
    void *dst;
    int64_t outer;
    int64_t src_cols;
    int64_t row_bytes;
} dc_gather_desc;
#define DC_GATHER_MAX_TENSORS 32
int dc_gather_columns(const dc_gather_desc *descs, int n_desc, const int64_t *index, int64_t n_index,
                      dc_stream_t stream);

size_t dc_rnn_workspace_bytes(int cell, int B, int H);
int dc_rnn_seq_fwd(int cell, float *gates, const float *w_hh, const float *b_hh, float *ybuf,
                   float *cbuf, int B, int S, int H, void *workspace, dc_stream_t stream);
int dc_rnn_seq_bwd(int cell, float *gates, const float *w_hh, const float *ybuf, float *cbuf,
                   const float *dy, const float *dhn, const float *dcn, float *dh0, float *dc0,
                   int B, int S, int H, void *workspace, dc_stream_t stream);

int dc_rnn_seq_fwd_reset(int cell, float *gates, const float *w_hh, const float *b_hh, float *ybuf, float *cbuf,
                         const int32_t *reset_slot, const float *reset_prev, const float *reset_pre, int K,
                         int B, int S, int H, void *workspace, dc_stream_t stream);
int dc_rnn_seq_bwd_reset(int cell, float *gates, const float *w_hh, const float *ybuf, float *cbuf,
                         const float *dy, const float *dhn, const float *dcn, float *dh0, float *dc0,
                         const int32_t *reset_slot, const float *reset_prev, int K,
                         int B, int S, int H, void *workspace, dc_stream_t stream);

int dc_gemm_tf32x3_supported(int64_t M, int N, int K);
int dc_gemm_tf32x3(const float *A, int lda, const float *B, int ldb, const float *bias, float *C, int ldc,
                   int64_t M, int N, int K, int relu, dc_stream_t stream);

size_t dc_gemm_wgrad_workspace_bytes(int No, int Ni);
int dc_gemm_wgrad_tf32x3(const float *dY, int ldy, const float *X, int ldx, int64_t T, int No, int Ni,
                         float *dW, int ldw, float *db, int accumulate, void *workspace, dc_stream_t stream);

size_t dc_unit_basic_bwd_workspace_bytes(void);
int dc_env_fwd(const float *env, const float *w_e, const float *b_e, float *out, int ld_out, int64_t N,
               dc_stream_t stream);
size_t dc_env_bwd_workspace_bytes(void);
int dc_env_bwd(const float *d_out, const float *out, int ld, const float *env, float *dw_e, float *db_e, int64_t N,
               void *workspace, dc_stream_t stream);
int dc_gemm_unit_max(const float *basic, const float *w, const float *bias, float *xmax, float *xmax_copy, int ld_x,
                     uint8_t *argmax, int64_t n_tokens, int n_units, dc_stream_t stream);
int dc_unit_embed_fwd(const float *units, const float *w_b, const float *b_b, float *basic_out, const float *w, const float *bias,
                      float *xmax, float *xmax_copy, int ld_x, uint8_t *argmax, int64_t n_tokens, int n_units, dc_stream_t stream);
int dc_target_unit_q_fwd(const float *q, int ld_q, const float *const units[6], const float *w_b, const float *b_b, float *logits,
                         int64_t N, dc_stream_t stream);
int dc_target_unit_q_bwd(const float *dlogits, const float *const units[6], const float *w_b, const float *b_b, float *s, int ld_s,
                         int64_t N, dc_stream_t stream);
int dc_unit_wgrad_routed(const float *d_xmax, const float *d_xmax2, int ld_dx, const uint8_t *argmax, const float *basic,
                         int64_t n_tokens, int n_units, float *dW, float *db, void *workspace, dc_stream_t stream);
int dc_unit_dgrad_fused(const float *d_xmax, const float *d_xmax2, int ld_dx, const uint8_t *argmax, const float *dlogits,
                        int ld_dl, const float *att, const float *w_t, const float *units, const float *w_b,
                        const float *b_b, int64_t n_tokens, int n_units, float *dw_b, float *db_b, int accumulate,
                        void *workspace, dc_stream_t stream);

#define DC_PPO_WORKSPACE_BYTES 512
int dc_ppo_loss_fwd_bwd(const float *const logits[DC_NUM_HEADS],
                        const uint8_t *const masks[DC_NUM_HEADS],
                        const uint8_t *const actions[DC_NUM_HEADS], const float *old_logp,
                        const float *adv_raw, const float *ret, const float *value, int64_t N,
                        float e_clip, float entropy_coef, float vf_coef,
                        float *const dlogits[DC_NUM_HEADS], float *dvalue, float *out,
                        int32_t *n_actions, void *workspace, dc_stream_t stream);

int dc_ppo_loss_fwd_bwd_strided(const float *const logits[DC_NUM_HEADS], const int64_t ld_logits[DC_NUM_HEADS],
                                const uint8_t *const masks[DC_NUM_HEADS],
                                const uint8_t *const actions[DC_NUM_HEADS], const float *old_logp,
                                const float *adv_raw, const float *ret, const float *value, int64_t ld_value,
                                int64_t N, float e_clip, float entropy_coef, float vf_coef,
                                float *const dlogits[DC_NUM_HEADS], const int64_t ld_dlogits[DC_NUM_HEADS],
                                float *dvalue, int64_t ld_dvalue, float *out, int32_t *n_actions,
                                void *workspace, dc_stream_t stream);

#define DC_HPARAM_SLOTS 8
#define DC_HP_LR 0
#define DC_HP_E_CLIP 1
#define DC_HP_ENTROPY_COEF 2
#define DC_HP_VF_COEF 3
#define DC_HP_MAX_GRAD_NORM 4
#define DC_HP_VALUE_CLIP 5

#define DC_PPO_STATS_SLOTS 16
#define DC_STAT_APPROX_KL 0
#define DC_STAT_CLIP_FRACTION 6
#define DC_STAT_EXPLAINED_VAR 12
#define DC_STAT_JOINT_APPROX_KL 13
#define DC_STAT_JOINT_CLIP_FRACTION 14
int dc_ppo_loss_fwd_bwd_dev(const float *const logits[DC_NUM_HEADS], const int64_t ld_logits[DC_NUM_HEADS],
                            const uint8_t *const masks[DC_NUM_HEADS],
                            const uint8_t *const actions[DC_NUM_HEADS], const float *old_logp,
                            const float *adv_raw, const float *ret, const float *value, int64_t ld_value,
                            const float *old_value, int64_t N, const double *hparams,
                            float *const dlogits[DC_NUM_HEADS], const int64_t ld_dlogits[DC_NUM_HEADS],
                            float *dvalue, int64_t ld_dvalue, float *out, float *stats, int32_t *n_actions,
                            void *workspace, dc_stream_t stream);

int dc_ppo_loss_fwd_bwd_masked(const float *const logits[DC_NUM_HEADS], const int64_t ld_logits[DC_NUM_HEADS],
                               const uint8_t *const masks[DC_NUM_HEADS],
                               const uint8_t *const actions[DC_NUM_HEADS], const float *old_logp,
                               const float *adv_raw, const float *ret, const float *value, int64_t ld_value,
                               const float *old_value, const uint8_t *valid, int64_t N, const double *hparams,
                               float *const dlogits[DC_NUM_HEADS], const int64_t ld_dlogits[DC_NUM_HEADS],
                               float *dvalue, int64_t ld_dvalue, float *out, float *stats, int32_t *n_actions,
                               void *workspace, dc_stream_t stream);

int dc_ppo_loss_fwd_bwd_joint(const float *const logits[DC_NUM_HEADS], const int64_t ld_logits[DC_NUM_HEADS],
                              const uint8_t *const masks[DC_NUM_HEADS],
                              const uint8_t *const actions[DC_NUM_HEADS], const float *old_logp,
                              const float *adv_raw, const float *ret, const float *value, int64_t ld_value,
                              const float *old_value, const uint8_t *valid, int64_t N, const double *hparams,
                              float *const dlogits[DC_NUM_HEADS], const int64_t ld_dlogits[DC_NUM_HEADS],
                              float *dvalue, int64_t ld_dvalue, float *out, float *stats, int32_t *n_actions,
                              void *workspace, dc_stream_t stream);

int dc_selected_logp(const float *const logits[DC_NUM_HEADS],
                     const uint8_t *const masks[DC_NUM_HEADS],
                     const uint8_t *const actions[DC_NUM_HEADS], int64_t N, float *logp_out,
                     dc_stream_t stream);

int dc_grad_flags(float *flat_grad, int64_t total, const int32_t *seg_head, int n_seg,
                  const int32_t *n_actions, dc_stream_t stream);
int dc_grad_finish(float *flat_param, float *flat_grad, float *exp_avg, float *exp_avg_sq,
                   int32_t *steps, const int64_t *seg_lo, const int64_t *seg_hi, const int32_t *seg_head, int n_seg,
                   int64_t total, double lr, double beta1, double beta2, double adam_eps,
                   double max_norm, const float *loss_out, float *metrics, void *workspace,
                   dc_stream_t stream);
int dc_grad_finish_dev(float *flat_param, float *flat_grad, float *exp_avg, float *exp_avg_sq,
                       int32_t *steps, const int64_t *seg_lo, const int64_t *seg_hi, const int32_t *seg_head, int n_seg,
                       int64_t total, const double *hparams, double beta1, double beta2, double adam_eps,
                       const float *loss_out, float *metrics, void *workspace, dc_stream_t stream);
#define DC_FINISH_WORKSPACE_BYTES 1024

int dc_select_actions(const float *const logits[DC_NUM_HEADS], const int64_t ld[DC_NUM_HEADS],
                      const uint8_t *const masks[DC_NUM_HEADS], const float *u, int64_t A, int32_t *chosen,
                      float *logp, dc_stream_t stream);

#ifdef __cplusplus
}
#endif
#endif
```

Baseline: 71.50.

## Save ReLU masks in forward and move unit dgrad weight reduction onto wgmma

The forward unit-embedding GEMM now writes a 128-bit ReLU activation mask per row, and the backward pass reads it instead of recomputing the basic unit embedding for every row and column. The dgrad kernel is restructured. W^T is kept resident in shared memory, the ring streams only the gradient tiles, and the per-column scalar FMA reduction over rows becomes a second tf32x3 wgmma (m64n16) against swizzled unit tiles, with the mask applied in registers. This removes heavy per-thread CUDA-core work and repeated weight loads, at the cost of extra mask memory traffic, more shared memory use and more complex synchronisation.

```diff
diff --git a/dotaclient_b200/_lib.py b/dotaclient_b200/_lib.py
--- a/dotaclient_b200/_lib.py
+++ b/dotaclient_b200/_lib.py
@@ -35,8 +35,11 @@
     "dc_env_bwd": (_i32, [_vp, _vp, _i32, _vp, _vp, _vp, _i64, _vp, _vp]),
     "dc_unit_wgrad_routed": (_i32, [_vp, _vp, _i32, _vp, _vp, _i64, _i32, _vp, _vp, _vp, _vp]),
     "dc_unit_dgrad_fused": (_i32, [_vp, _vp, _i32, _vp, _vp, _i32, _vp, _vp, _vp, _vp, _vp, _i64, _i32, _vp, _vp, _i32, _vp, _vp]),
+    "dc_unit_dgrad_fused_mask": (_i32, [_vp, _vp, _i32, _vp, _vp, _i32, _vp, _vp, _vp, _vp, _vp, _vp, _i64, _i32, _vp, _vp, _i32, _vp,
+                                        _vp]),
     "dc_gemm_unit_max": (_i32, [_vp, _vp, _vp, _vp, _vp, _i32, _vp, _i64, _i32, _vp]),
     "dc_unit_embed_fwd": (_i32, [_vp, _vp, _vp, _vp, _vp, _vp, _vp, _vp, _i32, _vp, _i64, _i32, _vp]),
+    "dc_unit_embed_fwd_mask": (_i32, [_vp, _vp, _vp, _vp, _vp, _vp, _vp, _vp, _vp, _i32, _vp, _i64, _i32, _vp]),
     "dc_target_unit_q_fwd": (_i32, [_vp, _i32, _c.c_void_p * 6, _vp, _vp, _vp, _i64, _vp]),
     "dc_target_unit_q_bwd": (_i32, [_vp, _c.c_void_p * 6, _vp, _vp, _vp, _i32, _i64, _vp]),
     "dc_ppo_loss_fwd_bwd": (_i32, [_ptr5, _ptr5, _ptr5, _vp, _vp, _vp, _vp, _i64, _f32, _f32, _f32, _ptr5, _vp, _vp,
diff --git a/dotaclient_b200/csrc/capi.cu b/dotaclient_b200/csrc/capi.cu
--- a/dotaclient_b200/csrc/capi.cu
+++ b/dotaclient_b200/csrc/capi.cu
@@ -25,7 +25,7 @@
 
 extern "C" {
 
-int dc_version(void) { return 107; }
+int dc_version(void) { return 108; }
 
 const char *dc_last_error(void) { return g_err; }
 
diff --git a/dotaclient_b200/csrc/gemm_tf32x3.cu b/dotaclient_b200/csrc/gemm_tf32x3.cu
--- a/dotaclient_b200/csrc/gemm_tf32x3.cu
+++ b/dotaclient_b200/csrc/gemm_tf32x3.cu
@@ -15,8 +15,7 @@
 constexpr int kLdS = BN + 8;
 constexpr int kDIn = kUnitFeatures;
 constexpr size_t kOffStaging = (size_t)kStages * kStageBytes;
-constexpr size_t kOffUnits = kOffStaging + (size_t)BM * kLdS * 4;
-constexpr size_t kOffBars = kOffUnits + (size_t)BM * kDIn * 4;
+constexpr size_t kOffBars = kOffStaging + (size_t)BM * kLdS * 4;
 constexpr size_t kSmemBytes = kOffBars + 128 + 1024 ;
 
 #define DC_ACC8(b) "+f"(d[b]), "+f"(d[b + 1]), "+f"(d[b + 2]), "+f"(d[b + 3]), "+f"(d[b + 4]), "+f"(d[b + 5]), "+f"(d[b + 6]), "+f"(d[b + 7])
@@ -320,6 +319,7 @@
 struct GenA {
     const float *units, *w_b, *b_b;
     float *basic_out;
+    uint32_t *mask_out;
 };
 
 __device__ __forceinline__ void cp_async16(uint32_t dst, const void *src, uint32_t src_bytes) {
@@ -473,6 +473,7 @@
     for (int mb = mb0; mb < m_blocks; mb += mstride, ++i, c += k_chunks) {
         if ((i & 1) != wg) continue;
         const int m0 = mb * kTileRows;
+        uint32_t mask_lo = 0, mask_hi = 0;
 #pragma unroll
         for (int j = 0; j < 64; ++j) d[j] = 0.f;
         float v[16];
@@ -503,6 +504,19 @@
                 wgmma_m64n128k8_rs(d, ahi[4 * ks], ahi[4 * ks + 1], ahi[4 * ks + 2], ahi[4 * ks + 3], b_hi + adv);
             }
             dc_wgmma_commit();
+            if (kGenA && gen.mask_out != nullptr) {
+                uint32_t lo = 0, hi = 0;
+#pragma unroll
+                for (int ks = 0; ks < BK / 8; ++ks) {
+#pragma unroll
+                    for (int h = 0; h < 2; ++h) {
+                        lo |= v[4 * ks + 2 * h] > 0.f ? 1u << (2 * ks + h) : 0u;
+                        hi |= v[4 * ks + 2 * h + 1] > 0.f ? 1u << (2 * ks + h) : 0u;
+                    }
+                }
+                mask_lo |= lo << (8 * kc);
+                mask_hi |= hi << (8 * kc);
+            }
             if (kc + 1 < k_chunks) {
                 const uint32_t cn = c + kc + 1;
                 const int s = cn % kWsStages;
@@ -514,6 +528,10 @@
             for (int j = 0; j < 16; ++j) asm volatile("" : "+r"(ahi[j]), "+r"(alo[j])::"memory");
 #pragma unroll
             for (int j = 0; j < 64; ++j) dc_reg_fence(d[j]);
+        }
+        if (kGenA && gen.mask_out != nullptr) {
+            if (m0 + rlo < M) gen.mask_out[(size_t)(m0 + rlo) * 4 + q] = mask_lo;
+            if (hi_ok && m0 + rhi < M) gen.mask_out[(size_t)(m0 + rhi) * 4 + q] = mask_hi;
         }
 
         if constexpr (NU == 0) {
@@ -567,81 +585,225 @@
     }
 }
 
-template <int NU>
-__global__ void __launch_bounds__(kThreads, 1) unit_dgrad_fused_kernel(const float *__restrict__ dx, const float *__restrict__ dx2, int ld_dx,
-                                                                       const uint8_t *__restrict__ argmax,
-                                                                       const float *__restrict__ dl, int ld_dl,
-                                                                       const float *__restrict__ att,
-                                                                       const float *__restrict__ Wt, const float *__restrict__ units,
-                                                                       const float *__restrict__ w_b, const float *__restrict__ b_b,
-                                                                       int n_tok, float *__restrict__ partial) {
+constexpr int kDgN = 16;
+constexpr int kDgUTile = kDgN * BK * 4;
+constexpr int kDgStageBytes = 2 * kTileBytes;
+constexpr size_t kDgOffRing = (size_t)(BN / BK) * 2 * kTileBytes;
+constexpr size_t kDgOffU = kDgOffRing + (size_t)kStages * kDgStageBytes;
+constexpr int kDgMaskLd = BM + 8;
+constexpr size_t kDgOffMask = kDgOffU + (size_t)2 * (BM / BK) * kDgUTile;
+constexpr size_t kDgOffWb = kDgOffMask + (size_t)4 * kDgMaskLd * 4;
+constexpr size_t kDgOffBars = kDgOffWb + (size_t)BN * (kDIn + 1) * 4;
+constexpr size_t kDgSmemBytes = kDgOffBars + 2 * (kStages + 1) * 8 + 1024 ;
+static_assert(kDgSmemBytes <= 227 * 1024, "unit data-gradient kernel exceeds the shared-memory opt-in");
+static_assert(kDgOffU % 1024 == 0 && kDgUTile % 1024 == 0, "the swizzled U tiles need 1024-byte alignment");
+
+__device__ __forceinline__ void wgmma_wait1() { asm volatile("wgmma.wait_group.sync.aligned 1;" ::: "memory"); }
+
+__device__ __forceinline__ void wgmma_m64n16k8_rs(float (&d)[8], const uint32_t (&a)[4], uint64_t desc_b) {
+    asm volatile(
+        "{\n\t.reg .pred p;\n\tsetp.ne.b32 p, %13, 0;\n\t"
+        "wgmma.mma_async.sync.aligned.m64n16k8.f32.tf32.tf32 {%0, %1, %2, %3, %4, %5, %6, %7}, {%8, %9, %10, %11}, %12, p, 1, 1;\n\t}\n"
+        : "+f"(d[0]), "+f"(d[1]), "+f"(d[2]), "+f"(d[3]), "+f"(d[4]), "+f"(d[5]), "+f"(d[6]), "+f"(d[7])
+        : "r"(a[0]), "r"(a[1]), "r"(a[2]), "r"(a[3]), "l"(desc_b), "r"(1));
+}
+
+struct DgAux {
+    float4 u[3];
+    uint32_t m[4];
+    bool ok;
+};
+
+template <bool kMask>
+__device__ __forceinline__ void aux_fetch(DgAux &x, const float *__restrict__ units, const uint32_t *__restrict__ mask, int m0,
+                                          int rows_valid, int t) {
+    const float4 zero4 = make_float4(0.f, 0.f, 0.f, 0.f);
+    x.ok = t < rows_valid;
+    const size_t row = (size_t)(m0 + (x.ok ? t : 0));
+#pragma unroll
+    for (int i = 0; i < 3; ++i) x.u[i] = x.ok ? __ldg(reinterpret_cast<const float4 *>(units) + row * 3 + i) : zero4;
+    if constexpr (kMask) {
+        const uint4 w = x.ok ? __ldg(reinterpret_cast<const uint4 *>(mask) + row) : make_uint4(0u, 0u, 0u, 0u);
+        x.m[0] = w.x; x.m[1] = w.y; x.m[2] = w.z; x.m[3] = w.w;
+    }
+}
+
+__device__ __forceinline__ void aux_recompute_mask(DgAux &x, const float *sw, const float *sb) {
+    const float u[kDIn] = {x.u[0].x, x.u[0].y, x.u[0].z, x.u[0].w, x.u[1].x, x.u[1].y, x.u[1].z, x.u[1].w, x.u[2].x, x.u[2].y, x.u[2].z, x.u[2].w};
+#pragma unroll
+    for (int w = 0; w < 4; ++w) {
+        uint32_t bits = 0;
+#pragma unroll 4
+        for (int i = 0; i < 32; ++i) {
+            const int j = 4 * i + w;
+            const float4 *wr4 = reinterpret_cast<const float4 *>(sw + j * kDIn);
+            const float4 w0 = wr4[0], w1 = wr4[1], w2 = wr4[2];
+            const float wr[kDIn] = {w0.x, w0.y, w0.z, w0.w, w1.x, w1.y, w1.z, w1.w, w2.x, w2.y, w2.z, w2.w};
+            bits |= (dc_unit_basic(u, wr, sb[j]) > 0.f ? 1u : 0u) << i;
+        }
+        x.m[w] = x.ok ? bits : 0u;
+    }
+}
+
+__device__ __forceinline__ void aux_store(const DgAux &x, unsigned char *sm_u, uint32_t *sm_mask, int t) {
+    const int k = 8 * (t >> 3) + ((t & 7) >> 1) + 4 * (t & 1), kk = k & 31;
+    unsigned char *base = sm_u + (k >> 5) * kDgUTile + (kk & 3) * 4;
+    const float v[kDgN] = {x.u[0].x, x.u[0].y, x.u[0].z, x.u[0].w, x.u[1].x, x.u[1].y, x.u[1].z, x.u[1].w,
+                           x.u[2].x, x.u[2].y, x.u[2].z, x.u[2].w, x.ok ? 1.f : 0.f, 0.f, 0.f, 0.f};
+#pragma unroll
+    for (int n = 0; n < kDgN; ++n) {
+        const float hi = dc_tf32_rna(v[n]);
+        const int off = n * 128 + (((kk >> 2) ^ (n & 7)) << 4);
+        *reinterpret_cast<float *>(base + off) = hi;
+        *reinterpret_cast<float *>(base + (BM / BK) * kDgUTile + off) = v[n] - hi;
+    }
+#pragma unroll
+    for (int w = 0; w < 4; ++w) sm_mask[w * kDgMaskLd + t] = x.m[w];
+}
+
+template <int NU, bool kMask>
+__global__ void __launch_bounds__(kThreads, 1) unit_dgrad_kernel(const float *__restrict__ dx, const float *__restrict__ dx2, int ld_dx,
+                                                                 const uint8_t *__restrict__ argmax,
+                                                                 const float *__restrict__ dl, int ld_dl,
+                                                                 const float *__restrict__ att,
+                                                                 const float *__restrict__ Wt, const float *__restrict__ units,
+                                                                 const uint32_t *__restrict__ mask,
+                                                                 const float *__restrict__ w_b, const float *__restrict__ b_b,
+                                                                 int n_tok, float *__restrict__ partial) {
     constexpr int kTileRows = BM - BM % NU, kTileToks = kTileRows / NU;
     constexpr int k_chunks = BN / BK;
     extern __shared__ unsigned char smem_raw[];
-    unsigned char *tiles = smem_base(smem_raw);
-    float *S = reinterpret_cast<float *>(tiles + kOffStaging);
-    float *U = reinterpret_cast<float *>(tiles + kOffUnits);
-    uint64_t *full = reinterpret_cast<uint64_t *>(tiles + kOffBars), *empty = full + kStages;
+    unsigned char *sm = smem_base(smem_raw);
+    unsigned char *ring = sm + kDgOffRing, *sm_u = sm + kDgOffU;
+    uint32_t *sm_mask = reinterpret_cast<uint32_t *>(sm + kDgOffMask);
+    float *sm_wb = reinterpret_cast<float *>(sm + kDgOffWb), *sm_bb = sm_wb + BN * kDIn;
+    uint64_t *full = reinterpret_cast<uint64_t *>(sm + kDgOffBars), *empty = full + kStages;
+    uint64_t *ufull = empty + kStages, *uempty = ufull + 1;
 
     const int warp = threadIdx.x >> 5, lane = threadIdx.x & 31;
     const int M = n_tok * NU;
     const int m_blocks = (M + kTileRows - 1) / kTileRows;
+    if constexpr (!kMask) {
+        for (int i = threadIdx.x; i < BN * kDIn; i += kThreads) sm_wb[i] = __ldg(w_b + i);
+        for (int i = threadIdx.x; i < BN; i += kThreads) sm_bb[i] = __ldg(b_b + i);
+    }
+    if (threadIdx.x == 0) {
+        dc_mbar_init(ufull, 4);
+        dc_mbar_init(uempty, kConsumerThreads / 32);
+    }
     init_ring(full);
 
     if (warp < kConsumerWarp0) {
         const int t = threadIdx.x & (kProducerThreads - 1), g = warp >> 2;
         uint32_t c = 0;
-        for (int mb = blockIdx.x; mb < m_blocks; mb += gridDim.x) {
-            const int tok0 = mb * kTileToks;
+        int it = 0;
+        for (int mb = blockIdx.x; mb < m_blocks; mb += gridDim.x, ++it) {
+            const int tok0 = mb * kTileToks, m0 = mb * kTileRows;
             for (int kc = 0; kc < k_chunks; ++kc, ++c) {
                 if ((int)(c % kProducerGroups) != g) continue;
                 DembRaw<NU> raw;
-                float4 vb[8];
+                DgAux aux;
                 demb_fetch<NU>(raw, dx, dx2, ld_dx, argmax, dl, ld_dl, att, tok0, n_tok, kc * BK, t);
-                tile_load_k(Wt, BN, 0, BN, kc * BK, t, vb);
-                produce(full, empty, c, lane, [&](int s) {
-                    unsigned char *st = tiles + (size_t)s * kStageBytes;
-                    demb_store<NU>(raw, st, st + kTileBytes, t);
-                    tile_store_k(vb, st + 2 * kTileBytes, st + 3 * kTileBytes, t);
-                });
+                if (kc == 0) aux_fetch<kMask>(aux, units, mask, m0, min(kTileRows, M - m0), t);
+                produce(full, empty, c, lane, [&](int s) { demb_store<NU>(raw, ring + (size_t)s * kDgStageBytes, ring + (size_t)s * kDgStageBytes + kTileBytes, t); });
+                if (kc == 0) {
+                    if constexpr (!kMask) aux_recompute_mask(aux, sm_wb, sm_bb);
+                    dc_mbar_wait(uempty, (it & 1) ^ 1);
+                    aux_store(aux, sm_u, sm_mask, t);
+                    asm volatile("fence.proxy.async.shared::cta;" ::: "memory");
+                    __syncwarp();
+                    if (lane == 0) dc_mbar_arrive(ufull);
+                }
             }
         }
     } else {
-        const int ct = threadIdx.x - kConsumerWarp0 * 32, wg = ct >> 7;
-        const int col = ct & (BN - 1), half = ct >> 7;
-        float wb[kDIn];
-#pragma unroll
-        for (int k = 0; k < kDIn; ++k) wb[k] = __ldg(w_b + col * kDIn + k);
-        const float bb = __ldg(b_b + col);
-        float acc[kDIn];
-#pragma unroll
-        for (int k = 0; k < kDIn; ++k) acc[k] = 0.f;
-        float accb = 0.f;
+        const int ct = threadIdx.x - kConsumerWarp0 * 32, wg = ct >> 7, w4 = (ct >> 5) & 3, t = ct & 127, q4 = lane & 3;
+        for (int kc = wg; kc < k_chunks; kc += 2) {
+            float4 vb[8];
+            tile_load_k(Wt, BN, 0, BN, kc * BK, t, vb);
+            tile_store_k(vb, sm + (size_t)kc * 2 * kTileBytes, sm + (size_t)kc * 2 * kTileBytes + kTileBytes, t);
+        }
+        asm volatile("fence.proxy.async.shared::cta;" ::: "memory");
+        consumer_sync();
+        const uint32_t w_base = dc_smem_u32(sm) + wg * (64 * 128), ring_base = dc_smem_u32(ring), u_base = dc_smem_u32(sm_u);
+        const int j_lo = 64 * wg + 16 * w4 + (lane >> 2);
+        const uint32_t bit_lo = 1u << (j_lo >> 2), bit_hi = bit_lo << 2;
+        const uint32_t *mrow = sm_mask + (j_lo & 3) * kDgMaskLd + 2 * q4;
+        float acc[8];
+#pragma unroll
+        for (int i = 0; i < 8; ++i) acc[i] = 0.f;
         float d[64];
         uint32_t c = 0;
-        for (int mb = blockIdx.x; mb < m_blocks; mb += gridDim.x) {
-            const int m0 = mb * kTileRows, rows_valid = min(kTileRows, M - m0);
-            consume(d, tiles, full, empty, c, k_chunks, wg, lane);
-            consumer_sync();
-            stage_acc(d, S, ct);
-            const float4 *usrc = reinterpret_cast<const float4 *>(units + (size_t)m0 * kDIn);
-            for (int i = ct; i < rows_valid * (kDIn / 4); i += kConsumerThreads) reinterpret_cast<float4 *>(U)[i] = __ldg(usrc + i);
-            consumer_sync();
-            const int r_end = min(64 * half + 64, rows_valid);
-            for (int r = 64 * half; r < r_end; ++r) {
-                const float4 *up = reinterpret_cast<const float4 *>(U + r * kDIn);
-                const float4 u0 = up[0], u1 = up[1], u2 = up[2];
-                const float u[kDIn] = {u0.x, u0.y, u0.z, u0.w, u1.x, u1.y, u1.z, u1.w, u2.x, u2.y, u2.z, u2.w};
-                const float gval = dc_unit_basic(u, wb, bb) > 0.f ? S[r * kLdS + col] : 0.f;
-#pragma unroll
-                for (int k = 0; k < kDIn; ++k) acc[k] = fmaf(gval, u[k], acc[k]);
-                accb += gval;
-            }
-        }
-        float *prow = partial + ((size_t)(blockIdx.x * 2 + half) * BN + col) * (kDIn + 1);
-#pragma unroll
-        for (int k = 0; k < kDIn; ++k) prow[k] = acc[k];
-        prow[kDIn] = accb;
+        int it = 0;
+        for (int mb = blockIdx.x; mb < m_blocks; mb += gridDim.x, ++it) {
+#pragma unroll
+            for (int i = 0; i < 64; ++i) d[i] = 0.f;
+#pragma unroll 1
+            for (int kc = 0; kc < k_chunks; ++kc, ++c) {
+                const int s = c % kStages;
+                dc_mbar_wait(&full[s], (c / kStages) & 1);
+#pragma unroll
+                for (int i = 0; i < 64; ++i) dc_reg_fence(d[i]);
+                dc_wgmma_fence();
+                const uint64_t a_hi = dc_wgmma_desc(w_base + kc * 2 * kTileBytes), a_lo = dc_wgmma_desc(w_base + kc * 2 * kTileBytes + kTileBytes);
+                const uint64_t b_hi = dc_wgmma_desc(ring_base + s * kDgStageBytes), b_lo = dc_wgmma_desc(ring_base + s * kDgStageBytes + kTileBytes);
+#pragma unroll
+                for (int ks = 0; ks < BK / 8; ++ks) {
+                    const uint64_t adv = (uint64_t)(ks * 2);
+                    wgmma_m64n128k8(d, a_hi + adv, b_lo + adv);
+                    wgmma_m64n128k8(d, a_lo + adv, b_hi + adv);
+                    wgmma_m64n128k8(d, a_hi + adv, b_hi + adv);
+                }
+                dc_wgmma_commit();
+                if (kc > 0) {
+                    wgmma_wait1();
+                    __syncwarp();
+                    if (lane == 0) dc_mbar_arrive(&empty[(c - 1) % kStages]);
+                }
+            }
+            dc_wgmma_wait0();
+#pragma unroll
+            for (int i = 0; i < 64; ++i) dc_reg_fence(d[i]);
+            __syncwarp();
+            if (lane == 0) dc_mbar_arrive(&empty[(c - 1) % kStages]);
+
+            dc_mbar_wait(ufull, it & 1);
+            uint32_t ghi[2][4], glo[2][4];
+#pragma unroll
+            for (int q = 0; q < BM / 8; ++q) {
+                const int b = q & 1;
+                const uint2 mw = *reinterpret_cast<const uint2 *>(mrow + 8 * q);
+                const float gv[4] = {(mw.x & bit_lo) ? d[4 * q] : 0.f, (mw.x & bit_hi) ? d[4 * q + 2] : 0.f,
+                                     (mw.y & bit_lo) ? d[4 * q + 1] : 0.f, (mw.y & bit_hi) ? d[4 * q + 3] : 0.f};
+#pragma unroll
+                for (int e = 0; e < 4; ++e) {
+                    const float h = dc_tf32_rna(gv[e]);
+                    ghi[b][e] = __float_as_uint(h);
+                    glo[b][e] = __float_as_uint(gv[e] - h);
+                }
+                dc_wgmma_fence();
+                const uint64_t u_hi = dc_wgmma_desc(u_base + (q >> 2) * kDgUTile) + 2 * (q & 3);
+                const uint64_t u_lo = dc_wgmma_desc(u_base + (BM / BK + (q >> 2)) * kDgUTile) + 2 * (q & 3);
+                wgmma_m64n16k8_rs(acc, glo[b], u_hi);
+                wgmma_m64n16k8_rs(acc, ghi[b], u_lo);
+                wgmma_m64n16k8_rs(acc, ghi[b], u_hi);
+                dc_wgmma_commit();
+                wgmma_wait1();
+#pragma unroll
+                for (int e = 0; e < 4; ++e) asm volatile("" : "+r"(ghi[b ^ 1][e]), "+r"(glo[b ^ 1][e])::"memory");
+            }
+            dc_wgmma_wait0();
+#pragma unroll
+            for (int i = 0; i < 8; ++i) dc_reg_fence(acc[i]);
+            __syncwarp();
+            if (lane == 0) dc_mbar_arrive(uempty);
+        }
+        float *pp = partial + (size_t)blockIdx.x * BN * (kDIn + 1);
+#pragma unroll
+        for (int i = 0; i < 8; ++i) {
+            const int j = j_lo + 8 * ((i >> 1) & 1), n = 8 * (i >> 2) + 2 * q4 + (i & 1);
+            if (n <= kDIn) pp[j * (kDIn + 1) + n] = acc[i];
+        }
     }
 }
 
@@ -654,7 +816,6 @@
 static_assert(kWgStageBytes % 1024 == 0, "the swizzled dY^T tiles need 1024-byte aligned slots");
 static_assert(kWgSmemBytes <= 227 * 1024, "weight-gradient GEMM exceeds the shared-memory opt-in");
 
-__device__ __forceinline__ void wgmma_wait1() { asm volatile("wgmma.wait_group.sync.aligned 1;" ::: "memory"); }
 __device__ __forceinline__ float lds_f32(uint32_t addr) {
     float v;
     asm volatile("ld.shared.f32 %0, [%1];" : "=f"(v) : "r"(addr) : "memory");
@@ -938,29 +1099,35 @@
     return launch_ws<16>(basic, BN, w, BN, bias, xmax, ld_x, M, BN, BN, 0, xmax_copy, argmax, st);
 }
 
-extern "C" int dc_unit_embed_fwd(const float *units, const float *w_b, const float *b_b, float *basic_out, const float *w, const float *bias,
-                                 float *xmax, float *xmax_copy, int ld_x, uint8_t *argmax, int64_t n_tokens, int n_units,
-                                 dc_stream_t stream) {
+extern "C" int dc_unit_embed_fwd_mask(const float *units, const float *w_b, const float *b_b, float *basic_out, uint32_t *mask_out,
+                                      const float *w, const float *bias, float *xmax, float *xmax_copy, int ld_x, uint8_t *argmax,
+                                      int64_t n_tokens, int n_units, dc_stream_t stream) {
     DC_REQUIRE(units && w_b && b_b && w && bias && xmax && n_tokens > 0, DC_EINVAL, "dc_unit_embed_fwd: null pointer / empty input");
     DC_REQUIRE(n_units == 1 || n_units == 5 || n_units == 16, DC_EUNSUPPORTED, "dc_unit_embed_fwd: n_units=%d (1, 5 or 16)", n_units);
     DC_REQUIRE(n_units == 1 ? (argmax == nullptr && xmax_copy == nullptr) : argmax != nullptr, DC_EINVAL,
                "dc_unit_embed_fwd: the arg-max (and the copy) go with the max-pool of n_units 5 and 16 only");
     DC_REQUIRE(ld_x >= BN && ld_x % 4 == 0 && n_tokens * n_units < (1ll << 31) - BM, DC_EINVAL, "dc_unit_embed_fwd: bad ld_x / size");
     DC_REQUIRE(((uintptr_t)units & 15) == 0 && ((uintptr_t)basic_out & 15) == 0 && ((uintptr_t)w & 15) == 0 && ((uintptr_t)bias & 15) == 0 &&
-                   ((uintptr_t)xmax & 15) == 0 && ((uintptr_t)xmax_copy & 15) == 0,
-               DC_EINVAL, "dc_unit_embed_fwd: units, basic_out, w, bias, xmax, xmax_copy must be 16-byte aligned");
+                   ((uintptr_t)xmax & 15) == 0 && ((uintptr_t)xmax_copy & 15) == 0 && ((uintptr_t)mask_out & 15) == 0,
+               DC_EINVAL, "dc_unit_embed_fwd: units, basic_out, mask_out, w, bias, xmax, xmax_copy must be 16-byte aligned");
     const int M = (int)(n_tokens * n_units);
-    const GenA gen{units, w_b, b_b, basic_out};
+    const GenA gen{units, w_b, b_b, basic_out, mask_out};
     cudaStream_t st = dc_cu_stream(stream);
     if (n_units == 1) return launch_ws<0, true>(nullptr, BN, w, BN, bias, xmax, ld_x, M, BN, BN, 0, nullptr, nullptr, st, gen);
     if (n_units == 5) return launch_ws<5, true>(nullptr, BN, w, BN, bias, xmax, ld_x, M, BN, BN, 0, xmax_copy, argmax, st, gen);
     return launch_ws<16, true>(nullptr, BN, w, BN, bias, xmax, ld_x, M, BN, BN, 0, xmax_copy, argmax, st, gen);
 }
 
-extern "C" int dc_unit_dgrad_fused(const float *d_xmax, const float *d_xmax2, int ld_dx, const uint8_t *argmax, const float *dlogits,
-                                   int ld_dl, const float *att, const float *w_t, const float *units, const float *w_b,
-                                   const float *b_b, int64_t n_tokens, int n_units, float *dw_b, float *db_b, int accumulate,
-                                   void *workspace, dc_stream_t stream) {
+extern "C" int dc_unit_embed_fwd(const float *units, const float *w_b, const float *b_b, float *basic_out, const float *w, const float *bias,
+                                 float *xmax, float *xmax_copy, int ld_x, uint8_t *argmax, int64_t n_tokens, int n_units,
+                                 dc_stream_t stream) {
+    return dc_unit_embed_fwd_mask(units, w_b, b_b, basic_out, nullptr, w, bias, xmax, xmax_copy, ld_x, argmax, n_tokens, n_units, stream);
+}
+
+extern "C" int dc_unit_dgrad_fused_mask(const float *d_xmax, const float *d_xmax2, int ld_dx, const uint8_t *argmax, const float *dlogits,
+                                        int ld_dl, const float *att, const float *w_t, const float *units, const uint32_t *mask,
+                                        const float *w_b, const float *b_b, int64_t n_tokens, int n_units, float *dw_b, float *db_b,
+                                        int accumulate, void *workspace, dc_stream_t stream) {
     DC_REQUIRE(w_t && units && w_b && b_b && dw_b && db_b && workspace && n_tokens > 0, DC_EINVAL, "dc_unit_dgrad_fused: null pointer / empty input");
     DC_REQUIRE(n_units == 1 || n_units == 5 || n_units == 16, DC_EUNSUPPORTED, "dc_unit_dgrad_fused: n_units=%d (1, 5 or 16)", n_units);
     DC_REQUIRE((d_xmax == nullptr && d_xmax2 == nullptr) || (d_xmax != nullptr && ld_dx >= BN && ld_dx % 4 == 0), DC_EINVAL,
@@ -970,26 +1137,40 @@
                "dc_unit_dgrad_fused: dlogits and att come together");
     DC_REQUIRE(n_tokens * n_units < (1ll << 31) - BM, DC_EINVAL, "dc_unit_dgrad_fused: too many rows");
     DC_REQUIRE(((uintptr_t)d_xmax & 15) == 0 && ((uintptr_t)d_xmax2 & 15) == 0 && ((uintptr_t)argmax & 3) == 0 && ((uintptr_t)att & 15) == 0 &&
-                   ((uintptr_t)w_t & 15) == 0 && ((uintptr_t)units & 15) == 0 && ((uintptr_t)workspace & 15) == 0,
-               DC_EINVAL, "dc_unit_dgrad_fused: d_xmax, att, w_t, units must be 16-byte aligned (arg-max 4-byte)");
+                   ((uintptr_t)w_t & 15) == 0 && ((uintptr_t)units & 15) == 0 && ((uintptr_t)mask & 15) == 0 && ((uintptr_t)workspace & 15) == 0,
+               DC_EINVAL, "dc_unit_dgrad_fused: d_xmax, att, w_t, units, mask must be 16-byte aligned (arg-max 4-byte)");
     const int n_tok = (int)n_tokens;
     const int tile_rows = BM - BM % n_units;
     int grid = (int)((n_tokens * n_units + tile_rows - 1) / tile_rows);
     if (grid > dc_sm_count()) grid = dc_sm_count();
     float *partial = reinterpret_cast<float *>(workspace);
     cudaStream_t st = dc_cu_stream(stream);
-#define DC_LAUNCH_DGRAD(NU)                                                                                                          \
+#define DC_LAUNCH_DGRAD(NU, MASK)                                                                                                    \
     do {                                                                                                                              \
-        DC_CUDA(cudaFuncSetAttribute(unit_dgrad_fused_kernel<NU>, cudaFuncAttributeMaxDynamicSharedMemorySize, (int)kSmemBytes)); \
-        unit_dgrad_fused_kernel<NU><<<grid, kThreads, kSmemBytes, st>>>(d_xmax, d_xmax2, ld_dx, argmax, dlogits, ld_dl, att, w_t,    \
-                                                                            units, w_b, b_b, n_tok, partial);                        \
+        DC_CUDA(cudaFuncSetAttribute(unit_dgrad_kernel<NU, MASK>, cudaFuncAttributeMaxDynamicSharedMemorySize, (int)kDgSmemBytes)); \
+        unit_dgrad_kernel<NU, MASK><<<grid, kThreads, kDgSmemBytes, st>>>(d_xmax, d_xmax2, ld_dx, argmax, dlogits, ld_dl, att, w_t,  \
+                                                                          units, mask, w_b, b_b, n_tok, partial);                     \
     } while (0)
-    if (n_units == 1) DC_LAUNCH_DGRAD(1);
-    else if (n_units == 5) DC_LAUNCH_DGRAD(5);
-    else DC_LAUNCH_DGRAD(16);
+    if (mask != nullptr) {
+        if (n_units == 1) DC_LAUNCH_DGRAD(1, true);
+        else if (n_units == 5) DC_LAUNCH_DGRAD(5, true);
+        else DC_LAUNCH_DGRAD(16, true);
+    } else {
+        if (n_units == 1) DC_LAUNCH_DGRAD(1, false);
+        else if (n_units == 5) DC_LAUNCH_DGRAD(5, false);
+        else DC_LAUNCH_DGRAD(16, false);
+    }
 #undef DC_LAUNCH_DGRAD
     DC_LAUNCH_OK();
-    return dc_unit_basic_reduce(partial, 2 * grid, dw_b, db_b, accumulate, st);
+    return dc_unit_basic_reduce(partial, grid, dw_b, db_b, accumulate, st);
+}
+
+extern "C" int dc_unit_dgrad_fused(const float *d_xmax, const float *d_xmax2, int ld_dx, const uint8_t *argmax, const float *dlogits,
+                                   int ld_dl, const float *att, const float *w_t, const float *units, const float *w_b,
+                                   const float *b_b, int64_t n_tokens, int n_units, float *dw_b, float *db_b, int accumulate,
+                                   void *workspace, dc_stream_t stream) {
+    return dc_unit_dgrad_fused_mask(d_xmax, d_xmax2, ld_dx, argmax, dlogits, ld_dl, att, w_t, units, nullptr, w_b, b_b, n_tokens, n_units,
+                                    dw_b, db_b, accumulate, workspace, stream);
 }
 
 extern "C" int dc_unit_wgrad_routed(const float *d_xmax, const float *d_xmax2, int ld_dx, const uint8_t *argmax, const float *basic,
diff --git a/dotaclient_b200/encoder_ops.py b/dotaclient_b200/encoder_ops.py
--- a/dotaclient_b200/encoder_ops.py
+++ b/dotaclient_b200/encoder_ops.py
@@ -80,7 +80,7 @@
             wait(env2)
         with PROFILE.span("env_fwd", 1, 4 * N * (3 + C)):
             _lib.check(lib.dc_env_fwd(env2.data_ptr(), w_e.data_ptr(), b_e.data_ptr(), xcat.data_ptr(), XCAT, N, st), "dc_env_fwd")
-        basics = []
+        basics, masks = [], []
         for g, n_u in enumerate(UNITS):
             R = N * n_u
             if wait is not None:
@@ -88,26 +88,28 @@
             if g == 5:
                 continue
             basic = torch.empty((R, C), dtype=torch.float32, device=dev) if need_grad else None
+            mask = torch.empty((R, 4), dtype=torch.int32, device=dev) if need_grad else None
             copy = _ptr(xcat, 6 * C) if g == 3 else None
             am = argmax[g].data_ptr() if n_u > 1 else None
-            nbytes = 4 * (R * 12 + (R * C if need_grad else 0) + C * C + N * C) + (N * C if n_u > 1 else 0)
+            nbytes = 4 * (R * 12 + (R * C + R * 4 if need_grad else 0) + C * C + N * C) + (N * C if n_u > 1 else 0)
             with PROFILE.span("gemm_unit_max" if n_u > 1 else "gemm_tf32x3", 1, nbytes):
-                _lib.check(lib.dc_unit_embed_fwd(units[g].data_ptr(), w_b.data_ptr(), b_b.data_ptr(), _lib.ptr(basic),
-                                                 weights[g].data_ptr(), biases[g].data_ptr(), _ptr(xcat, (g + 1) * C), copy, XCAT,
-                                                 am, N, n_u, st), "dc_unit_embed_fwd")
+                _lib.check(lib.dc_unit_embed_fwd_mask(units[g].data_ptr(), w_b.data_ptr(), b_b.data_ptr(), _lib.ptr(basic), _lib.ptr(mask),
+                                                      weights[g].data_ptr(), biases[g].data_ptr(), _ptr(xcat, (g + 1) * C), copy, XCAT,
+                                                      am, N, n_u, st), "dc_unit_embed_fwd_mask")
             basics.append(basic)
+            masks.append(mask)
         link["units"], link["w_b"], link["b_b"] = units, w_b, b_b
         link["weights"], link["biases"] = weights, biases
         ctx.N = N
         ctx.lead = lead
-        ctx.save_for_backward(argmax, *units, *basics, *weights, env2, xcat, w_b, b_b)
+        ctx.save_for_backward(argmax, *units, *basics, *weights, env2, xcat, w_b, b_b, *masks)
         return xcat.view(*lead, XCAT)
 
     @staticmethod
     def backward(ctx, d_xcat):
         saved = ctx.saved_tensors
         argmax, units, basics, weights, env2, xcat = saved[0], saved[1:7], saved[7:12], saved[12:18], saved[18], saved[19]
-        w_b, b_b = saved[20], saved[21]
+        w_b, b_b, masks = saved[20], saved[21], saved[22:27]
         N = ctx.N
         lib = _lib.load()
         st = _lib.stream_ptr()
@@ -143,12 +145,14 @@
                     _lib.check(lib.dc_gemm_wgrad_tf32x3(dx, XCAT, basics[g].data_ptr(), C, R, C, C, dw_all[g].data_ptr(), C,
                                                         db_all[g].data_ptr(), 0, ws_w.data_ptr(), st), "dc_gemm_wgrad_tf32x3")
             wt = weights[g].t().contiguous()
-            with PROFILE.span("unit_dgrad_fused", 2, N * (4 * C + C) * (1 if routed else 0) + 4 * R * 12 + (4 * N * (C + n_u) if dl is not None else 0)):
-                _lib.check(lib.dc_unit_dgrad_fused(dx, dx2, XCAT, argmax[g].data_ptr() if (routed and n_u > 1) else None,
-                                                   None if dl is None else _ptr(dl, off), MAX_UNITS, None if att is None else att.data_ptr(),
-                                                   wt.data_ptr(), units[g].data_ptr(), w_b.data_ptr(), b_b.data_ptr(), N, n_u,
-                                                   dw_b.data_ptr(), db_b.data_ptr(), 1 if g > 0 else 0, ws_b.data_ptr(), st),
-                           "dc_unit_dgrad_fused")
+            mask = masks[g] if routed else None
+            with PROFILE.span("unit_dgrad_fused", 2, N * (4 * C + C) * (1 if routed else 0) + 4 * R * 12 + (16 * R if routed else 0)
+                              + (4 * N * (C + n_u) if dl is not None else 0)):
+                _lib.check(lib.dc_unit_dgrad_fused_mask(dx, dx2, XCAT, argmax[g].data_ptr() if (routed and n_u > 1) else None,
+                                                        None if dl is None else _ptr(dl, off), MAX_UNITS, None if att is None else att.data_ptr(),
+                                                        wt.data_ptr(), units[g].data_ptr(), _lib.ptr(mask), w_b.data_ptr(), b_b.data_ptr(),
+                                                        N, n_u, dw_b.data_ptr(), db_b.data_ptr(), 1 if g > 0 else 0, ws_b.data_ptr(), st),
+                           "dc_unit_dgrad_fused_mask")
         if dl is not None:
             dw_head = torch.empty((C, QW), dtype=torch.float32, device=dev)
             with PROFILE.span("gemm_wgrad", 2, 4 * (N * C + N * QW + C * QW)):
diff --git a/include/dotaclient_b200.h b/include/dotaclient_b200.h
--- a/include/dotaclient_b200.h
+++ b/include/dotaclient_b200.h
@@ -78,6 +78,9 @@
                      uint8_t *argmax, int64_t n_tokens, int n_units, dc_stream_t stream);
 int dc_unit_embed_fwd(const float *units, const float *w_b, const float *b_b, float *basic_out, const float *w, const float *bias,
                       float *xmax, float *xmax_copy, int ld_x, uint8_t *argmax, int64_t n_tokens, int n_units, dc_stream_t stream);
+int dc_unit_embed_fwd_mask(const float *units, const float *w_b, const float *b_b, float *basic_out, uint32_t *mask_out, const float *w,
+                           const float *bias, float *xmax, float *xmax_copy, int ld_x, uint8_t *argmax, int64_t n_tokens, int n_units,
+                           dc_stream_t stream);
 int dc_target_unit_q_fwd(const float *q, int ld_q, const float *const units[6], const float *w_b, const float *b_b, float *logits,
                          int64_t N, dc_stream_t stream);
 int dc_target_unit_q_bwd(const float *dlogits, const float *const units[6], const float *w_b, const float *b_b, float *s, int ld_s,
@@ -88,6 +91,10 @@
                         int ld_dl, const float *att, const float *w_t, const float *units, const float *w_b,
                         const float *b_b, int64_t n_tokens, int n_units, float *dw_b, float *db_b, int accumulate,
                         void *workspace, dc_stream_t stream);
+int dc_unit_dgrad_fused_mask(const float *d_xmax, const float *d_xmax2, int ld_dx, const uint8_t *argmax, const float *dlogits,
+                             int ld_dl, const float *att, const float *w_t, const float *units, const uint32_t *mask, const float *w_b,
+                             const float *b_b, int64_t n_tokens, int n_units, float *dw_b, float *db_b, int accumulate,
+                             void *workspace, dc_stream_t stream);
 
 #define DC_PPO_WORKSPACE_BYTES 512
 int dc_ppo_loss_fwd_bwd(const float *const logits[DC_NUM_HEADS],
```

After: 78.37 (median of 6 runs). +9.6%, better.
